# voxelmorph/voxelmorph

Hardware: NVIDIA H100
Metric: vol-pairs/sec (3D 160x192x224 VxmDense int_steps=7 train step, NCC+Grad, Adam) (higher is better)
Workload: dtype bf16 (conv operands) / f32 (accumulate, warp, VecInt, losses)

## Files before the change

include/vxm_b200.h:

```cpp
#ifndef VXM_B200_H
#define VXM_B200_H

#include <stddef.h>
#include <stdint.h>

#ifdef __cplusplus
extern "C" {
#endif

#define VXM_OK 0
#define VXM_ERR_ARG (-1)
#define VXM_ERR_CUDA (-2)
#define VXM_ERR_UNSUPPORTED (-3)

#define VXM_MODE_LINEAR 0
#define VXM_MODE_NEAREST 1
#define VXM_ARITH_TRUE_DIV 0
#define VXM_ARITH_RECIPROCAL 1
#define VXM_ARITH_FAST 2

const char* vxm_last_error(void);
const char* vxm_version(void);
uint64_t vxm_launch_count(void);

int vxm_warp_fwd(const float* src, const float* flow, float* out,
                 int B, int C, int Ds, int Hs, int Ws, int D, int H, int W, int nd,
                 int mode, int arith, void* stream);
int vxm_warp_bwd(const float* grad_out, const float* src, const float* flow,
                 float* grad_src, float* grad_flow,
                 int B, int C, int Ds, int Hs, int Ws, int D, int H, int W, int nd,
                 int mode, int arith, void* stream);

size_t vxm_vecint_workspace_bytes(int B, int D, int H, int W, int nd, int nsteps);
int vxm_vecint_fwd(const float* vel, float* out, float* states, void* work,
                   int B, int D, int H, int W, int nd, int nsteps, int arith, void* stream);
int vxm_vecint_bwd(const float* grad_out, const float* states, float* grad_vel, void* work,
                   int B, int D, int H, int W, int nd, int nsteps, int arith, void* stream);
size_t vxm_vecint_fast_states_bytes(int B, int D, int H, int W, int nsteps);
size_t vxm_vecint_fast_work_bytes(int B, int D, int H, int W, int backward);
int vxm_debug_gridsync(int nsync, int ctas_per_sm, void* stream);

int vxm_resize_fwd(const float* x, float* out, int B, int C, int Di, int Hi, int Wi,
                   int Do, int Ho, int Wo, float pre, float post, void* stream);
int vxm_resize_bwd(const float* grad_out, float* grad_x, int B, int C, int Di, int Hi, int Wi,
                   int Do, int Ho, int Wo, float pre, float post, void* stream);

int vxm_ncc_fwd(const float* I, const float* J, float* loss, float* saved, void* work,
                int B, int D, int H, int W, int wd, int wh, int ww, void* stream);
int vxm_ncc_bwd(const float* I, const float* J, const float* saved, const float* grad_loss,
                float* grad_J, int B, int D, int H, int W, int wd, int wh, int ww, void* stream);
int vxm_ncc_fwd2(const float* I, const float* J, float* loss, float* saved, void* work, int which,
                 int B, int D, int H, int W, int wd, int wh, int ww, void* stream);
int vxm_ncc_bwd2(const float* I, const float* J, const float* saved, const float* grad_loss, float* grad_I,
                 float* grad_J, int which, int B, int D, int H, int W, int wd, int wh, int ww, void* stream);

int vxm_jacdet(const float* disp, float* det, unsigned long long* folds, int B, int D, int H, int W, int nd, void* stream);

size_t vxm_reduce_workspace_bytes(void);
int vxm_gradloss_fwd(const float* y, float* loss, void* work, int B, int C, int D, int H, int W,
                     int nd, int penalty, float mult, void* stream);
int vxm_gradloss_bwd(const float* y, const float* grad_loss, float* grad_y, int B, int C, int D,
                     int H, int W, int nd, int penalty, float mult, void* stream);

int vxm_mse_fwd(const float* y_true, const float* y_pred, float* loss, void* work, size_t n,
                void* stream);
int vxm_mse_bwd(const float* y_true, const float* y_pred, const float* grad_loss,
                float* grad_pred, size_t n, void* stream);
int vxm_mse_scaled_fwd(const float* y_true, const float* y_pred, float* loss, void* work, size_t n, double scale,
                       void* stream);
int vxm_mse_scaled_bwd(const float* y_true, const float* y_pred, const float* grad_loss, float* grad_pred, size_t n,
                       double scale, void* stream);

int vxm_kl_fwd(const float* params, float* loss, void* work, int B, int D, int H, int W, int nd, float prior_lambda,
               void* stream);
int vxm_kl_bwd(const float* params, const float* grad_loss, float* grad_params, int B, int D, int H, int W, int nd,
               float prior_lambda, void* stream);

size_t vxm_dice_workspace_bytes(int BL);
int vxm_dice_fwd(const float* y_true, const float* y_pred, float* loss, float* sums, void* work,
                 int BL, size_t V, void* stream);
int vxm_dice_bwd(const float* y_true, const float* sums, const float* grad_loss, float* grad_pred,
                 int BL, size_t V, void* stream);

int vxm_conv3d_fwd_f32(const float* x, const float* w, const float* bias, float* y,
                       int B, int Cin, int Cout, int D, int H, int W, int kd,
                       float leaky_slope, void* stream);
size_t vxm_conv3d_bwd_workspace_bytes(int B, int Cin, int Cout, int D, int H, int W, int kd);
int vxm_conv3d_bwd_f32(const float* grad_y, const float* y, const float* x, const float* w,
                       float* grad_x, float* grad_w, float* grad_b, void* work,
                       int B, int Cin, int Cout, int D, int H, int W, int kd,
                       float leaky_slope, void* stream);

size_t vxm_conv3d_tc_packed_bytes(int cin_eff, int np, int kd);
int vxm_conv3d_tc_pack(const float* w, void* wpk, int Cout, int Cin, int kd, int np, int transposed,
                       void* stream);
int vxm_conv3d_tc_fwd(const void* xa, const void* xb, const float* const* xf, const long long* xf_bstride,
                      int nplanar, const void* wpk, const float* bias, void* out, const void* mask,
                      int B, int D, int H, int W, int Ca, int Cb, int up, int Cout, int np, int kd,
                      int out_mode, float slope, void* out2, int csplit, void* stream);
size_t vxm_conv3d_tct_packed_bytes(int cin_eff, int coutp, int kd);
int vxm_conv3d_tct_pack(const float* w, void* wpk, int Cout, int Cin, int kd, int coutp, int transposed, void* stream);
int vxm_conv3d_tct_supported(int Ca, int Cb, int Cout);
int vxm_conv3d_tct_fwd(const void* xa, const void* xb, const void* wpk, const float* bias, void* out, const void* mask,
                       int B, int D, int H, int W, int Ca, int Cb, int up, int Cout, int coutp, int kd, int out_mode,
                       float slope, void* out2, int csplit, void* stream);
size_t vxm_conv3d_tcs_packed_bytes(int cin_eff, int coutp, int kd);
int vxm_conv3d_tcs_pack(const float* w, void* wpk, int Cout, int Cin, int kd, int coutp, int transposed, void* stream);
int vxm_conv3d_tcs_supported(int Ca, int Cb, int Cout);
size_t vxm_conv3d_tcs_pack_desc_bytes(void);
int vxm_conv3d_tcs_pack_desc(void* desc_host, const float* w, void* wpk, int Cout, int Cin, int kd, int coutp, int transposed,
                             int begin);
int vxm_conv3d_tcs_pack_desc_blk(void* desc_host, const float* w, void* wpk, int Cout, int Cin, int kd, int coutp, int transposed,
                                 int n0, int nb, int k0, int kb, int begin);
int vxm_conv3d_tcs_pack_desc_fold(void* desc_host, const float* w, void* wpk, int Cout, int Cin, int coutp, int transposed, int begin);
int vxm_conv3d_tcs_pack_multi(const void* descs_dev, int ndesc, int total, void* stream);
int vxm_conv3d_tcs_fwd(const void* xa, const void* xb, const void* wpk, const float* bias, void* out, const void* mask,
                       int B, int D, int H, int W, int Ca, int Cb, int up, int Cout, int coutp, int kd, int out_mode,
                       float slope, void* out2, int csplit, void* stream);
int vxm_conv3d_tcs_fwd_acc(const void* xa, const void* xb, const void* wpk, const float* bias, void* out, void* out_lo,
                           const float* acc_in, int B, int D, int H, int W, int Ca, int Cb, int up, int Cout, int coutp,
                           int kd, int out_mode, float slope, void* stream);
int vxm_conv3d_tcs_fits(int cin, int coutp, int kd);
int vxm_conv3d_tcs_fwd_blk(const void* xa, const void* xb, const void* wpk, const float* bias, void* out, void* out_lo,
                           const void* mask, const float* acc_in, int B, int D, int H, int W, int Ca, int Cb, int up, int Cout,
                           int coutp, int kd, int out_mode, float slope, int opitch, void* stream);
size_t vxm_conv3d_tcs_poly_packed_bytes(int mode, int Cout, int Cin, int Ca);
int vxm_conv3d_tcs_pack_desc_poly(void* desc_host, const float* w, void* wpk, int Cout, int Cin, int Ca, int mode, int begin);
int vxm_conv3d_tcs_poly(const void* xa, const void* xb, const void* wpk, const float* bias, void* out, const void* mask, int B, int D,
                        int H, int W, int Ca, int Cb, int Cout, int mode, float slope, void* stream);
size_t vxm_conv3d_tc_wgrad_workspace_bytes(int kd);
int vxm_conv3d_tc_wgrad(const void* xa, const void* xb, const float* const* xf, const long long* xf_bstride,
                        int nplanar_x, const void* gz, const float* const* gf, const long long* gf_bstride,
                        int nplanar_g, float* grad_w, float* grad_b, void* work, int B, int D, int H, int W,
                        int Ca, int Cb, int up, int Cin_real, int Cg, int Cout_real, int kd, int accumulate, void* stream);
size_t vxm_conv3d_tc_wgrad2_desc_bytes(void);
int vxm_conv3d_tc_wgrad2_max_pending(void);
size_t vxm_conv3d_tc_wgrad2_partial_bytes(int kd);
int vxm_conv3d_tc_wgrad2_partial(const void* xa, const void* xb, const void* gz, float* grad_w, float* grad_b, void* work,
                                 size_t work_bytes, size_t* work_used, void* descs_host, int* ndesc, int B, int D, int H, int W,
                                 int Ca, int Cb, int up, int Cin_real, int Cg, int Cout_real, int kd, int accumulate, void* stream);
int vxm_conv3d_tc_wgrad2_flush(const void* descs_host, int ndesc, void* stream);
int vxm_conv3d_tc_wgrad2_partial_khm(const void* x, const void* gz, float* grad_w, float* grad_b, void* work, size_t work_bytes,
                                     size_t* work_used, void* descs_host, int* ndesc, int B, int D, int H, int W, int Cx,
                                     int Cin_real, int Cg, int Cout_real, int accumulate, void* stream);
int vxm_pool2_ndhwc_bf16(const void* x_fine, void* y_coarse, int B, int Dc, int Hc, int Wc, int C, int nd, void* stream);
int vxm_sumpool_mask_ndhwc_bf16(const void* g_fine, const void* act_coarse, void* out_coarse, int B, int Dc, int Hc,
                                int Wc, int C, int nd, float slope, void* stream);
int vxm_unpool_combine_ndhwc_bf16(const void* e_fine, const void* g_skip_fine, const void* g_pool_coarse, void* out_fine,
                                  int B, int Dc, int Hc, int Wc, int C, int nd, float slope, void* stream);
int vxm_planar_to_ndhwc8_bf16(const float* const* planes, const long long* bstrides, int nplanes, void* out, int B,
                              size_t V, void* stream);
int vxm_planar_fold_kd_bf16(const float* const* planes, const long long* bstrides, int nplanes, void* out, int B, int D,
                            size_t HW, int cout, void* stream);
int vxm_planar_to_ndhwc8_split_bf16(const float* const* planes, const long long* bstrides, int nplanes, void* out_hi,
                                    void* out_lo, int B, size_t V, void* stream);
int vxm_pool2_split_ndhwc_bf16(const void* x_hi, const void* x_lo, void* y_hi, void* y_lo, int B, int Dc, int Hc, int Wc,
                               int C, int nd, void* stream);
int vxm_unpool_combine_split_ndhwc_bf16(const void* e_hi, const void* e_lo, const void* g_skip_fine, const void* g_pool_coarse,
                                        void* out_fine, int B, int Dc, int Hc, int Wc, int C, int nd, float slope, void* stream);

int vxm_maxpool2_fwd(const float* x, float* y, uint8_t* idx, int B, int C, int D, int H, int W,
                     int nd, void* stream);
int vxm_maxpool2_bwd(const float* grad_y, const uint8_t* idx, float* grad_x, int B, int C, int D,
                     int H, int W, int nd, void* stream);
int vxm_upcat_fwd(const float* a, const float* skip, float* out, int B, int Ca, int Cb, int D,
                  int H, int W, int nd, void* stream);
int vxm_upcat_bwd(const float* grad_out, float* grad_a, float* grad_skip, int B, int Ca, int Cb,
                  int D, int H, int W, int nd, void* stream);

int vxm_adam_step(float* p, const float* g, float* m, float* v, size_t n, int step, float lr,
                  float beta1, float beta2, float eps, float weight_decay, float grad_scale,
                  void* stream);

int vxm_adam_step_dev(float* p, const float* g, float* m, float* v, size_t n, int* step_counter, float lr,
                      float beta1, float beta2, float eps, float weight_decay, float grad_scale, void* stream);

int vxm_mean_stream_fwd(const float* x, float* mean, float* count, float* out, float* saved, void* work, int B, size_t n,
                        float cap, int commit, void* stream);
int vxm_mean_stream_bwd(const float* grad_out, const float* saved, float* grad_x, int B, size_t n, size_t gout_bstride,
                        void* stream);

int vxm_sample_normal_logvar_fwd(const float* params, float* z, long long* state, long long* ticket, void* work, int B,
                                 int nd, size_t V, void* stream);
int vxm_sample_normal_logvar_bwd(const float* grad_z, const float* params, const long long* state, const long long* ticket,
                                 float* grad_params, int B, int nd, size_t V, void* stream);

size_t vxm_pheno_decoder_workspace_bytes(int F);
int vxm_pheno_decoder_fwd(const float* pheno, const float* W, const float* bias, const float* like_w, const float* like_b,
                          float* out, int B, int P, int F, size_t V, void* stream);
int vxm_pheno_decoder_bwd(const float* grad_out, const float* pheno, const float* W, const float* bias, const float* like_w,
                          float* grad_W, float* grad_bias, float* grad_like_w, float* grad_like_b, void* work, int B, int P,
                          int F, size_t V, int accumulate, void* stream);

size_t vxm_hyper_workspace_bytes(int U, size_t N);
int vxm_hyper_mlp_fwd(const float* hyp, const float* const* weights, const float* const* biases, float* pre, float* h,
                      int P, int U, int nb_layers, void* stream);
int vxm_hyper_mlp_bwd(const float* grad_h, const float* hyp, const float* const* weights, const float* pre,
                      float* const* grad_weights, float* const* grad_biases, int P, int U, int nb_layers, int accumulate,
                      void* stream);
int vxm_hyper_weights_fwd(const float* h, const float* A, const float* a, float* W, int U, size_t N, void* stream);
int vxm_hyper_weights_bwd(const float* h, const float* A, const float* grad_W, float* grad_A, float* grad_a,
                          float* grad_h, void* work, int U, size_t N, int accumulate, void* stream);

size_t vxm_mi_workspace_bytes(int N, size_t V, int nbins);
int vxm_mi_fwd(const float* y_true, const float* y_pred, const float* centers, float* loss, void* work, void* reduce_work,
               int N, size_t V, int nbins, float alpha, float min_clip, float max_clip, void* stream);
int vxm_mi_bwd(const float* y_true, const float* y_pred, const float* centers, const float* grad_loss, float* grad_true,
               float* grad_pred, void* work, int N, size_t V, int nbins, float alpha, float min_clip, float max_clip,
               void* stream);

size_t vxm_point_warp_workspace_bytes(int B, int N, int D, int H, int W, int nd);
int vxm_point_warp_fwd(const float* points, const float* flow, float* out, int B, int N, int D, int H, int W, int nd,
                       float r, void* stream);
int vxm_point_warp_bwd(const float* points, const float* grad_out, float* grad_flow, void* work, size_t work_bytes,
                       int B, int N, int D, int H, int W, int nd, float r, void* stream);
int vxm_value_at_fwd(const float* sdt, const float* points, float* out, int B, int N, int L, int D, int H, int W,
                     int nd, void* stream);
int vxm_value_at_bwd(const float* sdt, const float* points, const float* grad_out, float* grad_points, int B, int N,
                     int L, int D, int H, int W, int nd, void* stream);

#ifdef __cplusplus
}
#endif
#endif
```

voxelmorph_b200/_lib.py:

```python
import ctypes
import os
import threading

import torch

_HERE = os.path.dirname(os.path.abspath(__file__))
LIB_PATH = os.path.join(_HERE, "libvxm_b200.so")

c_f = ctypes.c_void_p
c_i = ctypes.c_int
c_sz = ctypes.c_size_t
c_fl = ctypes.c_float
c_d = ctypes.c_double

SIGNATURES = {
    "vxm_last_error": (ctypes.c_char_p, []),
    "vxm_version": (ctypes.c_char_p, []),
    "vxm_launch_count": (ctypes.c_uint64, []),
    "vxm_warp_fwd": (c_i, [c_f, c_f, c_f] + [c_i] * 9 + [c_i, c_i, c_f]),
    "vxm_warp_bwd": (c_i, [c_f, c_f, c_f, c_f, c_f] + [c_i] * 9 + [c_i, c_i, c_f]),
    "vxm_vecint_workspace_bytes": (c_sz, [c_i] * 6),
    "vxm_vecint_fwd": (c_i, [c_f, c_f, c_f, c_f] + [c_i] * 7 + [c_f]),
    "vxm_vecint_bwd": (c_i, [c_f, c_f, c_f, c_f] + [c_i] * 7 + [c_f]),
    "vxm_vecint_fast_states_bytes": (c_sz, [c_i] * 5),
    "vxm_vecint_fast_work_bytes": (c_sz, [c_i] * 5),
    "vxm_debug_gridsync": (c_i, [c_i, c_i, c_f]),
    "vxm_resize_fwd": (c_i, [c_f, c_f] + [c_i] * 8 + [c_fl, c_fl, c_f]),
    "vxm_resize_bwd": (c_i, [c_f, c_f] + [c_i] * 8 + [c_fl, c_fl, c_f]),
    "vxm_ncc_fwd": (c_i, [c_f, c_f, c_f, c_f, c_f] + [c_i] * 7 + [c_f]),
    "vxm_ncc_bwd": (c_i, [c_f, c_f, c_f, c_f, c_f] + [c_i] * 7 + [c_f]),
    "vxm_ncc_fwd2": (c_i, [c_f, c_f, c_f, c_f, c_f] + [c_i] * 8 + [c_f]),
    "vxm_ncc_bwd2": (c_i, [c_f, c_f, c_f, c_f, c_f, c_f] + [c_i] * 8 + [c_f]),
    "vxm_jacdet": (c_i, [c_f, c_f, c_f] + [c_i] * 5 + [c_f]),
    "vxm_reduce_workspace_bytes": (c_sz, []),
    "vxm_gradloss_fwd": (c_i, [c_f, c_f, c_f] + [c_i] * 7 + [c_fl, c_f]),
    "vxm_gradloss_bwd": (c_i, [c_f, c_f, c_f] + [c_i] * 7 + [c_fl, c_f]),
    "vxm_mse_fwd": (c_i, [c_f, c_f, c_f, c_f, c_sz, c_f]),
    "vxm_mse_bwd": (c_i, [c_f, c_f, c_f, c_f, c_sz, c_f]),
    "vxm_mse_scaled_fwd": (c_i, [c_f, c_f, c_f, c_f, c_sz, c_d, c_f]),
    "vxm_mse_scaled_bwd": (c_i, [c_f, c_f, c_f, c_f, c_sz, c_d, c_f]),
    "vxm_kl_fwd": (c_i, [c_f, c_f, c_f] + [c_i] * 5 + [c_fl, c_f]),
    "vxm_kl_bwd": (c_i, [c_f, c_f, c_f] + [c_i] * 5 + [c_fl, c_f]),
    "vxm_dice_workspace_bytes": (c_sz, [c_i]),
    "vxm_dice_fwd": (c_i, [c_f, c_f, c_f, c_f, c_f, c_i, c_sz, c_f]),
    "vxm_dice_bwd": (c_i, [c_f, c_f, c_f, c_f, c_i, c_sz, c_f]),
    "vxm_conv3d_fwd_f32": (c_i, [c_f, c_f, c_f, c_f] + [c_i] * 7 + [c_fl, c_f]),
    "vxm_conv3d_bwd_workspace_bytes": (c_sz, [c_i] * 7),
    "vxm_conv3d_bwd_f32": (c_i, [c_f] * 8 + [c_i] * 7 + [c_fl, c_f]),
    "vxm_conv3d_tc_packed_bytes": (c_sz, [c_i] * 3),
    "vxm_conv3d_tc_pack": (c_i, [c_f, c_f] + [c_i] * 5 + [c_f]),
    "vxm_conv3d_tc_fwd": (c_i, [c_f, c_f, c_f, c_f, c_i, c_f, c_f, c_f, c_f] + [c_i] * 11 + [c_fl, c_f, c_i, c_f]),
    "vxm_conv3d_tct_packed_bytes": (c_sz, [c_i] * 3),
    "vxm_conv3d_tct_pack": (c_i, [c_f, c_f] + [c_i] * 5 + [c_f]),
    "vxm_conv3d_tct_supported": (c_i, [c_i] * 3),
    "vxm_conv3d_tct_fwd": (c_i, [c_f, c_f, c_f, c_f, c_f, c_f] + [c_i] * 11 + [c_fl, c_f, c_i, c_f]),
    "vxm_conv3d_tcs_packed_bytes": (c_sz, [c_i] * 3),
    "vxm_conv3d_tcs_pack": (c_i, [c_f, c_f] + [c_i] * 5 + [c_f]),
    "vxm_conv3d_tcs_supported": (c_i, [c_i] * 3),
    "vxm_conv3d_tcs_pack_desc_bytes": (c_sz, []),
    "vxm_conv3d_tcs_pack_desc": (c_i, [c_f, c_f, c_f] + [c_i] * 6),
    "vxm_conv3d_tcs_pack_desc_blk": (c_i, [c_f, c_f, c_f] + [c_i] * 10),
    "vxm_conv3d_tcs_pack_desc_fold": (c_i, [c_f, c_f, c_f] + [c_i] * 5),
    "vxm_conv3d_tcs_pack_multi": (c_i, [c_f, c_i, c_i, c_f]),
    "vxm_conv3d_tcs_fwd": (c_i, [c_f, c_f, c_f, c_f, c_f, c_f] + [c_i] * 11 + [c_fl, c_f, c_i, c_f]),
    "vxm_conv3d_tcs_fwd_acc": (c_i, [c_f, c_f, c_f, c_f, c_f, c_f, c_f] + [c_i] * 11 + [c_fl, c_f]),
    "vxm_conv3d_tcs_fits": (c_i, [c_i] * 3),
    "vxm_conv3d_tcs_fwd_blk": (c_i, [c_f] * 8 + [c_i] * 11 + [c_fl, c_i, c_f]),
    "vxm_conv3d_tcs_poly_packed_bytes": (c_sz, [c_i] * 4),
    "vxm_conv3d_tcs_pack_desc_poly": (c_i, [c_f, c_f, c_f] + [c_i] * 5),
    "vxm_conv3d_tcs_poly": (c_i, [c_f] * 6 + [c_i] * 8 + [c_fl, c_f]),
    "vxm_conv3d_tc_wgrad_workspace_bytes": (c_sz, [c_i]),
    "vxm_conv3d_tc_wgrad": (c_i, [c_f, c_f, c_f, c_f, c_i, c_f, c_f, c_f, c_i, c_f, c_f, c_f] + [c_i] * 12 + [c_f]),
    "vxm_conv3d_tc_wgrad2_desc_bytes": (c_sz, []),
    "vxm_conv3d_tc_wgrad2_max_pending": (c_i, []),
    "vxm_conv3d_tc_wgrad2_partial_bytes": (c_sz, [c_i]),
    "vxm_conv3d_tc_wgrad2_partial": (c_i, [c_f, c_f, c_f, c_f, c_f, c_f, c_sz, c_f, c_f, c_f] + [c_i] * 12 + [c_f]),
    "vxm_conv3d_tc_wgrad2_flush": (c_i, [c_f, c_i, c_f]),
    "vxm_conv3d_tc_wgrad2_partial_khm": (c_i, [c_f, c_f, c_f, c_f, c_f, c_sz, c_f, c_f, c_f] + [c_i] * 9 + [c_f]),
    "vxm_pool2_ndhwc_bf16": (c_i, [c_f, c_f] + [c_i] * 6 + [c_f]),
    "vxm_sumpool_mask_ndhwc_bf16": (c_i, [c_f, c_f, c_f] + [c_i] * 6 + [c_fl, c_f]),
    "vxm_unpool_combine_ndhwc_bf16": (c_i, [c_f, c_f, c_f, c_f] + [c_i] * 6 + [c_fl, c_f]),
    "vxm_planar_to_ndhwc8_bf16": (c_i, [c_f, c_f, c_i, c_f, c_i, c_sz, c_f]),
    "vxm_planar_to_ndhwc8_split_bf16": (c_i, [c_f, c_f, c_i, c_f, c_f, c_i, c_sz, c_f]),
    "vxm_planar_fold_kd_bf16": (c_i, [c_f, c_f, c_i, c_f, c_i, c_i, c_sz, c_i, c_f]),
    "vxm_pool2_split_ndhwc_bf16": (c_i, [c_f, c_f, c_f, c_f] + [c_i] * 6 + [c_f]),
    "vxm_unpool_combine_split_ndhwc_bf16": (c_i, [c_f, c_f, c_f, c_f, c_f] + [c_i] * 6 + [c_fl, c_f]),
    "vxm_maxpool2_fwd": (c_i, [c_f, c_f, c_f] + [c_i] * 6 + [c_f]),
    "vxm_maxpool2_bwd": (c_i, [c_f, c_f, c_f] + [c_i] * 6 + [c_f]),
    "vxm_upcat_fwd": (c_i, [c_f, c_f, c_f] + [c_i] * 7 + [c_f]),
    "vxm_upcat_bwd": (c_i, [c_f, c_f, c_f] + [c_i] * 7 + [c_f]),
    "vxm_adam_step": (c_i, [c_f, c_f, c_f, c_f, c_sz, c_i] + [c_fl] * 6 + [c_f]),
    "vxm_adam_step_dev": (c_i, [c_f, c_f, c_f, c_f, c_sz, c_f] + [c_fl] * 6 + [c_f]),
    "vxm_mean_stream_fwd": (c_i, [c_f] * 6 + [c_i, c_sz, c_fl, c_i, c_f]),
    "vxm_mean_stream_bwd": (c_i, [c_f, c_f, c_f, c_i, c_sz, c_sz, c_f]),
    "vxm_sample_normal_logvar_fwd": (c_i, [c_f] * 5 + [c_i, c_i, c_sz, c_f]),
    "vxm_sample_normal_logvar_bwd": (c_i, [c_f] * 5 + [c_i, c_i, c_sz, c_f]),
    "vxm_pheno_decoder_workspace_bytes": (c_sz, [c_i]),
    "vxm_pheno_decoder_fwd": (c_i, [c_f] * 6 + [c_i, c_i, c_i, c_sz, c_f]),
    "vxm_pheno_decoder_bwd": (c_i, [c_f] * 10 + [c_i, c_i, c_i, c_sz, c_i, c_f]),
    "vxm_hyper_workspace_bytes": (c_sz, [c_i, c_sz]),
    "vxm_hyper_mlp_fwd": (c_i, [c_f] * 5 + [c_i, c_i, c_i, c_f]),
    "vxm_hyper_mlp_bwd": (c_i, [c_f] * 6 + [c_i, c_i, c_i, c_i, c_f]),
    "vxm_hyper_weights_fwd": (c_i, [c_f] * 4 + [c_i, c_sz, c_f]),
    "vxm_hyper_weights_bwd": (c_i, [c_f] * 7 + [c_i, c_sz, c_i, c_f]),
    "vxm_mi_workspace_bytes": (c_sz, [c_i, c_sz, c_i]),
    "vxm_mi_fwd": (c_i, [c_f] * 6 + [c_i, c_sz, c_i, c_fl, c_fl, c_fl, c_f]),
    "vxm_mi_bwd": (c_i, [c_f] * 7 + [c_i, c_sz, c_i, c_fl, c_fl, c_fl, c_f]),
    "vxm_point_warp_workspace_bytes": (c_sz, [c_i] * 6),
    "vxm_point_warp_fwd": (c_i, [c_f] * 3 + [c_i] * 6 + [c_fl, c_f]),
    "vxm_point_warp_bwd": (c_i, [c_f] * 4 + [c_sz] + [c_i] * 6 + [c_fl, c_f]),
    "vxm_value_at_fwd": (c_i, [c_f] * 3 + [c_i] * 7 + [c_f]),
    "vxm_value_at_bwd": (c_i, [c_f] * 4 + [c_i] * 7 + [c_f]),
}

_lib = None
_lock = threading.Lock()


class VxmError(RuntimeError):
    pass


def load():
    global _lib
    if _lib is not None:
        return _lib
    with _lock:
        if _lib is not None:
            return _lib
        if not os.path.isfile(LIB_PATH):
            raise VxmError(
                "voxelmorph_b200: %s not found — build it with `python -c 'import __graft_entry__ as g; g.build()'` "
                "(or `make -C voxelmorph_b200/csrc`).  There is no CPU / torch fallback." % LIB_PATH)
        lib = ctypes.CDLL(LIB_PATH)
        for name, (res, args) in SIGNATURES.items():
            fn = getattr(lib, name)
            fn.restype = res
            fn.argtypes = args
        _lib = lib
    return _lib


def last_error():
    return load().vxm_last_error().decode("utf-8", "replace")


def check(rc, what):
    if rc != 0:
        raise VxmError("%s failed (%d): %s" % (what, rc, last_error()))


def launch_count():
    return int(load().vxm_launch_count())


def ptr(t):
    if t is None:
        return None
    return ctypes.c_void_p(t.data_ptr())


def stream_ptr():
    return ctypes.c_void_p(torch.cuda.current_stream().cuda_stream)


def require_cuda(*tensors, what="voxelmorph_b200"):
    for t in tensors:
        if t is None:
            continue
        if not t.is_cuda:
            raise VxmError("%s: CUDA tensors are required (the GPU path has no CPU fallback); got a %s tensor"
                           % (what, t.device))
        if t.dtype != torch.float32:
            raise VxmError("%s: float32 tensors are required at the module boundary; got %s" % (what, t.dtype))


def contig(t):
    return t if t.is_contiguous() else t.contiguous()


_reduce_ws = {}


def reduce_workspace(device):
    key = (device.index, torch.cuda.current_stream(device).cuda_stream)
    ws = _reduce_ws.get(key)
    if ws is None:
        lib = load()
        with _lock:
            ws = _reduce_ws.get(key)
            if ws is None:
                nbytes = int(lib.vxm_reduce_workspace_bytes())
                ws = torch.zeros(nbytes, dtype=torch.uint8, device=device)
                _reduce_ws[key] = ws
    return ws
```

voxelmorph_b200/csrc/conv3d_tc_s.cu:

```cuda
#include <stdlib.h>
#include <string.h>

#include "tc_common.cuh"

namespace vxm {
namespace tcs {

using namespace vxm::tc;

constexpr int WT = 32, WUSE = 30;
constexpr int MAXSLOT = 16;
constexpr int NLOADER = 128, NTHREADS = 384, NGRP = 2;

struct ConvSArgs {
  const __nv_bfloat16* xa; const __nv_bfloat16* xb;
  const __nv_bfloat16* wpk; const float* bias;
  void* out; const __nv_bfloat16* mask;
  void* out2; int csplit;
  int B, D, H, W, Ca, Cb, up, upd, Cout, out_mode;
  float slope;
  int tiles_h, tiles_w, dchunk, nchunks, nitems, nslot;
  uint32_t wbytes;
  const float* acc_in; void* out_lo;
  int tma_mask, tc0[2];
  int opitch;
  alignas(64) CUtensorMap tm[2];
};

__host__ __device__ inline uint32_t swz(uint32_t off, uint32_t width) {
  return off ^ (((off >> 7) & (width / 16 - 1)) << 4);
}
__device__ __forceinline__ uint64_t make_desc_kmajor_swz(uint32_t saddr, uint32_t width) {
  uint64_t d = 0;
  d |= (uint64_t)((saddr >> 4) & 0x3FFF);
  d |= (uint64_t)1 << 16;
  d |= (uint64_t)(((8u * width) >> 4) & 0x3FFF) << 32;
  return d | desc_swizzle(width);
}

__device__ __forceinline__ void named_bar_arrive(int id, int nthreads) {
  asm volatile("bar.arrive %0, %1;" ::"r"(id), "r"(nthreads) : "memory");
}

template <int KD, int G0, int G1, int COUT, int HT, bool ACC, int EPI, bool OP = false, int PD = 0>
__global__ void __launch_bounds__(NTHREADS, 1) conv_tcs_kernel(const __grid_constant__ ConvSArgs a) {
  static_assert(PD == 0 || (KD == 3 && EPI != 0 && !ACC && !OP), "polyphase forms: 3-D, specialised epilogue");
  static_assert(PD != 1 || G1 > 0, "the polyphase forward merges channel group 0 and keeps group 1");
  static_assert(PD != 2 || (G1 == 0 && COUT == 32 && HT == 8 && EPI == 2), "the coarse dgrad: 32 -> 32 channels, 8-row tiles");
  static_assert(EPI != 4 || (PD == 0 && !ACC && !OP && COUT <= 32), "the fp32 planar epilogue drains in the fragment layout");
  static_assert(KD == 3 || EPI == 0 || (EPI != 3 && COUT <= 32), "KD = 1: fragment-layout epilogues 1, 2, 4 only");
  constexpr int SROWS = (HT + 2) * WT;
  constexpr int NH = PD == 2 ? 1 : HT / 4;
  constexpr int NEVEN = (HT + 3) / 2;
  constexpr int W0 = G0 * 2, W1 = G1 * 2;
  constexpr int NC8 = (G0 + G1) / 8;
  constexpr uint32_t SLAB0 = SROWS * W0, SLAB1 = SROWS * W1;
  constexpr int NN = 3 * COUT;
  extern __shared__ __align__(1024) uint8_t smem[];
  const bool halfk = (a.Ca + a.Cb == 8);
  constexpr uint32_t slab_bytes = SLAB0 + SLAB1;
  const int NSLOT = a.nslot;
  uint8_t* s_w = smem;
  uint8_t* s_slab = smem + ((a.wbytes + 1023u) & ~1023u);
  float* s_stage = reinterpret_cast<float*>(s_slab + NSLOT * slab_bytes);
  uint64_t* bars = reinterpret_cast<uint64_t*>(s_stage + NGRP * ACC_STAGE_FLOATS);
  uint64_t* full = bars;
  uint64_t* empty = bars + MAXSLOT;
  uint64_t* wbar = empty + MAXSLOT;

  const int warp = threadIdx.x >> 5, lane = threadIdx.x & 31;

  const bool tma0 = a.tma_mask & 1, tma1 = (a.tma_mask & 2) != 0;
  const bool all_tma = tma0 && (G1 == 0 || tma1);
  if (threadIdx.x == 0) {
    for (int i = 0; i < NSLOT; ++i) { mbar_init(&full[i], all_tma ? 1 : NLOADER); mbar_init(&empty[i], 4 * NGRP); }
    mbar_init(wbar, 1);
    fence_barrier_init();
  }
  __syncthreads();

  if (threadIdx.x == 0) {
    mbar_expect_tx(wbar, a.wbytes);
    for (uint32_t off = 0; off < a.wbytes; off += 16384u) {
      uint32_t n = a.wbytes - off < 16384u ? a.wbytes - off : 16384u;
      bulk_g2s(s_w + off, reinterpret_cast<const uint8_t*>(a.wpk) + off, n, wbar);
    }
  }
  const int HW_tiles = a.tiles_h * a.tiles_w;
  const int Dout = PD == 2 ? a.D >> 1 : a.D;

  if (warp >= 8) {
    const int lt = threadIdx.x - 8 * 32;
    uint32_t slot = 0, lphase = 1;
    const int Da = a.upd ? a.D >> 1 : a.D, Ha = a.up ? a.H >> 1 : a.H, Wa = a.up ? a.W >> 1 : a.W;
    const int nca8 = a.Ca >> 3;
    constexpr int nchunk = NC8 * SROWS;
    constexpr int KMAX = (nchunk + NLOADER - 1) / NLOADER;
    if (lt == 0) {
      if (tma0) tma_prefetch_desc(&a.tm[0]);
      if (tma1) tma_prefetch_desc(&a.tm[1]);
    }
    const uint32_t tma_bytes = (tma0 ? SLAB0 : 0u) + (tma1 ? SLAB1 : 0u);
    for (int item = blockIdx.x; item < a.nitems && !(all_tma && lt != 0); item += gridDim.x) {
      const int wt = item % a.tiles_w, ht = (item / a.tiles_w) % a.tiles_h;
      const int ch = (item / HW_tiles) % a.nchunks, b = item / (HW_tiles * a.nchunks);
      const int h0 = ht * HT, w0 = wt * WUSE, d0 = ch * a.dchunk, d1 = min(d0 + a.dchunk, Dout);
      const int s_begin = PD == 2 ? 2 * d0 - 1 : (KD == 3 ? d0 - 1 : d0), s_end = PD == 2 ? 2 * d1 + 1 : (KD == 3 ? d1 + 1 : d1);
      int soff[KMAX];
      uint32_t doff[KMAX];
#pragma unroll
      for (int k = 0; k < KMAX; ++k) {
        const int id = lt + k * NLOADER;
        soff[k] = -1;
        doff[k] = 0;
        if (id < nchunk) {
          const int c8 = id % NC8, row = id / NC8;
          const int r = row >> 5, c = row & 31;
          const int h = h0 - 1 + r, w = w0 - 1 + c;
          const int srow = PD == 2 ? ((r & 1) ? NEVEN + (r >> 1) : (r >> 1)) * WT + c : row;
          doff[k] = c8 < G0 / 8 ? swz((uint32_t)srow * W0 + (uint32_t)c8 * 16u, W0)
                                : SLAB0 + swz((uint32_t)row * W1 + (uint32_t)(c8 - G0 / 8) * 16u, W1 ? W1 : 32);
          if (c8 < G0 / 8 ? tma0 : tma1) soff[k] = -2;
          else if (h >= 0 && h < a.H && w >= 0 && w < a.W && !(halfk && c8 > 0)) {
            if (c8 < nca8) soff[k] = (((a.up ? h >> 1 : h) * Wa + (a.up ? w >> 1 : w)) * a.Ca + c8 * 8) << 1;
            else soff[k] = (((h * a.W + w) * a.Cb + (c8 - nca8) * 8) << 1) | 1;
          }
        }
      }
      for (int ds = s_begin; ds < s_end; ++ds) {
        mbar_wait(&empty[slot], lphase);
        uint8_t* slab = s_slab + (size_t)slot * slab_bytes;
        const bool dok = ds >= 0 && ds < a.D;
        const __nv_bfloat16* baseA = a.xa ? a.xa + (((size_t)b * Da + (dok ? (a.upd ? ds >> 1 : ds) : 0)) * Ha * Wa) * a.Ca : nullptr;
        const __nv_bfloat16* baseB = a.xb ? a.xb + (((size_t)b * a.D + (dok ? ds : 0)) * a.H * a.W) * a.Cb : nullptr;
        const __nv_bfloat16* dummy = a.xa ? a.xa : a.xb;
        if (lt == 0 && tma_bytes) {
          if (all_tma) mbar_expect_tx(&full[slot], tma_bytes);
          else mbar_expect_tx_noarrive(&full[slot], tma_bytes);
          if (tma0) tma_load_5d(slab, &a.tm[0], a.tc0[0], w0 - 1, h0 - 1, ds, b, &full[slot]);
          if (tma1) tma_load_5d(slab + SLAB0, &a.tm[1], a.tc0[1], w0 - 1, h0 - 1, ds, b, &full[slot]);
        }
        if (!all_tma) {
#pragma unroll
          for (int k = 0; k < KMAX; ++k) {
            if (lt + k * NLOADER < nchunk && soff[k] != -2) {
              const bool ok = dok && soff[k] >= 0;
              const __nv_bfloat16* src = ok ? ((soff[k] & 1) ? baseB : baseA) + (soff[k] >> 1) : dummy;
              cp_async16(slab + doff[k], src, ok ? 16u : 0u);
            }
          }
          cp_async_arrive_noinc(&full[slot]);
        }
        if (++slot == (uint32_t)NSLOT) { slot = 0; lphase ^= 1; }
      }
    }
  } else {
    const int grp = warp >> 2;
    const int wq = warp & 3;
    float* stage = s_stage + grp * ACC_STAGE_FLOATS;
    const int nbar = 1 + grp;
    constexpr int NSUB = NN > 96 ? 2 : 1;
    constexpr int NF = 2 / NSUB;
    constexpr int NCH = NSUB == 1 ? COUT / 16 : (COUT + 31) / 32;
    const int trow0 = NSUB == 1 ? wq : (wq & 1);
    auto chan = [&](int i) { return NSUB == 1 ? 16 * i : 32 * i + 16 * (wq >> 1); };
    const uint32_t slab_u32 = smem_u32(s_slab), w_u32 = smem_u32(s_w);
    constexpr uint32_t WSTEP = (uint32_t)NN * (W0 + W1);
    mbar_wait(wbar, 0);
    const uint64_t bdesc0 = make_desc_kmajor_swz(w_u32, W0);
    const uint64_t bdesc1 = make_desc_kmajor_swz(w_u32 + NN * W0, W1 ? W1 : 32);
    uint32_t cnt_base = 0, ecnt = 0, wcur = 0;
    auto observe = [&](uint32_t upto) {
      for (; wcur <= upto; ++wcur) mbar_wait(&full[wcur % NSLOT], (wcur / NSLOT) & 1);
    };
    constexpr int NKD = PD == 2 ? 4 : KD;
    auto mma = [&](uint32_t hslot, int hb, int sub, float (&acc)[NF][NN / 2], int par) {
      uint64_t adesc0_kd[NKD], adesc1_kd[NKD];
      uint32_t sl = hslot;
#pragma unroll
      for (int kd = 0; kd < NKD; ++kd) {
        adesc0_kd[kd] = make_desc_kmajor_swz(slab_u32 + sl * slab_bytes, W0);
        adesc1_kd[kd] = make_desc_kmajor_swz(slab_u32 + sl * slab_bytes + SLAB0, W1 ? W1 : 32);
        if (++sl == (uint32_t)NSLOT) sl = 0;
      }
      wg_fence();
#pragma unroll
      for (int kd = 0; kd < NKD; ++kd) {
#pragma unroll
        for (int kh = 0; kh < (PD == 2 ? 4 : 3); ++kh) {
          const int st = kd * (PD == 2 ? 4 : 3) + kh;
#pragma unroll
          for (int k = 0; k < (G0 + G1) / 16; ++k) {
            const bool g0 = k < G0 / 16;
            if (PD == 1 && g0 && kd == 2) continue;
            const int kk = g0 ? k : k - G0 / 16;
            const uint32_t wr = g0 ? W0 : W1;
            uint64_t abase = g0 ? adesc0_kd[kd] : adesc1_kd[kd];
            uint32_t wst = st * WSTEP;
            if (PD == 1 && g0 && par) {
              abase = adesc0_kd[kd + 1 < NKD ? kd + 1 : kd];
              wst = kd == 0 ? 9 * WSTEP + kh * NN * W0 : (6 + kh) * WSTEP;
            }
            const int r0 = PD == 2 ? ((kh & 1) ? NEVEN : 0) + (kh >> 1) : hb * 4 + kh;
            const uint64_t adesc = abase + (uint64_t)((r0 * WT * wr + kk * 32) >> 4);
            const uint64_t bdesc = (g0 ? bdesc0 : bdesc1) + (uint64_t)((wst + kk * 32) >> 4);
#pragma unroll
            for (int f = 0; f < NF; ++f)
              Wgmma<NN, 0, 0>::mma(acc[f], adesc + (uint64_t)(((sub + f) * 2 * WT * wr) >> 4), bdesc, (st | k) ? 1u : 0u);
          }
        }
      }
      wg_commit();
    };
    auto readout = [&](float (&acc)[NF][NN / 2], int c, uint32_t (&r)[16]) {
      if constexpr (NSUB == 1) acc_row16(acc[0], acc[NF - 1], c, stage, nbar, r);
      else acc_half_row16(acc[0], c, COUT - (c % COUT) < 32 ? 16 : 32, stage, nbar, r);
    };
    auto combine = [&](float (&acc)[NF][NN / 2], int i, float (&v)[16]) {
      const int cb = NSUB == 1 ? 16 * i : 32 * i;
      uint32_t r[16];
      readout(acc, cb, r);
#pragma unroll
      for (int c = 0; c < 16; ++c) v[c] = __shfl_up_sync(0xffffffffu, __uint_as_float(r[c]), 1);
      readout(acc, COUT + cb, r);
#pragma unroll
      for (int c = 0; c < 16; ++c) v[c] += __uint_as_float(r[c]);
      readout(acc, 2 * COUT + cb, r);
#pragma unroll
      for (int c = 0; c < 16; ++c) v[c] += __shfl_down_sync(0xffffffffu, __uint_as_float(r[c]), 1);
    };
    auto release = [&](int nd) {
      if (KD == 3) {
        const uint32_t last = PD == 2 ? 2u * nd : (uint32_t)nd;
        observe(cnt_base + last + 1u);
        if (lane == 0) {
          mbar_arrive(&empty[(cnt_base + last) % NSLOT]);
          mbar_arrive(&empty[(cnt_base + last + 1) % NSLOT]);
        }
        cnt_base += last + 2;
      } else {
        cnt_base += nd;
      }
    };
    if constexpr (EPI != 0) {
      const float slope = a.slope;
      const int c1 = (EPI == 3 && a.out2) ? a.csplit : COUT;
      const int Ho = PD == 2 ? a.H >> 1 : a.H, Wo = PD == 2 ? a.W >> 1 : a.W;
      const size_t HWp = (size_t)Ho * Wo;
      const int q = lane >> 2, p = lane & 3, half = wq & 1, pair = wq >> 1;
      const int xbar = 3 + 2 * grp + pair;
      constexpr bool ROWS = NSUB > 1 || PD == 2;
      constexpr int XPAIR = NF * 2 * COUT;
      static_assert(2 * 2 * XPAIR <= ACC_STAGE_FLOATS, "seam exchange fits the stage buffer");
      uint32_t xpar = 0;
      constexpr bool ORD = !ROWS;
      [[maybe_unused]] uint32_t nev = 0;
      if constexpr (ORD) {
        for (int item = blockIdx.x; item < a.nitems; item += gridDim.x) {
          const int d0 = ((item / HW_tiles) % a.nchunks) * a.dchunk;
          nev += (uint32_t)(min(d0 + a.dchunk, Dout) - d0) * NH;
        }
        if (grp == 1) named_bar_arrive(7, 256);
      }
      for (int item = blockIdx.x; item < a.nitems; item += gridDim.x) {
        const int wt = item % a.tiles_w, ht = (item / a.tiles_w) % a.tiles_h;
        const int ch = (item / HW_tiles) % a.nchunks, b = item / (HW_tiles * a.nchunks);
        const int d0 = ch * a.dchunk, d1 = min(d0 + a.dchunk, Dout);
        const int nd = d1 - d0;
        const int wp = 16 * half + q, w = wt * WUSE - 1 + wp;
        const int hbase = ht * HT + pair;
        uint32_t okm = 0;
#pragma unroll
        for (int hb = 0; hb < NH; ++hb)
#pragma unroll
          for (int blk = 0; blk < 2; ++blk)
#pragma unroll
            for (int i = 0; i < 2; ++i)
              if (wp + 8 * i >= 1 && wp + 8 * i <= WUSE && w + 8 * i < a.W && hbase + 4 * hb + 2 * blk < Ho)
                okm |= 1u << (4 * hb + 2 * blk + i);
        size_t vbase = (((size_t)b * Dout + d0) * Ho + hbase) * Wo + (size_t)(long long)w;
        [[maybe_unused]] const size_t DHWp = (size_t)Dout * HWp, pbase = (size_t)b * (a.Cout - 1) * DHWp;
        for (int j = 0; j < nd; ++j) {
          const uint32_t js = PD == 2 ? 2u * j : (uint32_t)j;
          observe(cnt_base + js + (PD == 2 ? 3u : (KD == 3 ? 2u : 0u)));
          const uint32_t hslot = (cnt_base + js) % NSLOT;
#pragma unroll
          for (int hb = 0; hb < NH; ++hb) {
            if ((int)(ecnt++ % NGRP) != grp) continue;
            auto vox_of = [&](int blk, int i) { return vbase + (size_t)((4 * hb + 2 * blk) * Wo + 8 * i); };
#pragma unroll
            for (int sub = 0; sub < NSUB; ++sub) {
              [[maybe_unused]] uint32_t mreg[EPI == 2 && !ROWS ? NF : 1][2][COUT / 8];
              auto load_mask = [&](int f) {
                if constexpr (EPI == 2 && !ROWS) {
#pragma unroll
                  for (int i = 0; i < 2; ++i)
                    if (okm >> (4 * hb + 2 * f + i) & 1u) {
                      const uint32_t* mp = reinterpret_cast<const uint32_t*>(a.mask + vox_of(f, i) * (OP ? a.opitch : COUT) + 2 * p);
#pragma unroll
                      for (int jj = 0; jj < COUT / 8; ++jj) mreg[f][i][jj] = __ldg(mp + 4 * jj);
                    }
                }
              };
              if constexpr (COUT == 16) {
#pragma unroll
                for (int f = 0; f < NF; ++f) load_mask(f);
              }
              const int rh = PD == 2 ? ht * (HT / 2) + trow0 : ht * HT + hb * 4 + trow0 + 2 * sub, rw = wt * WUSE - 1 + lane;
              const bool rvalid = lane >= 1 && lane <= WUSE && rw < a.W && rh < Ho && (PD != 2 || (lane & 1));
              const size_t rvox = (((size_t)b * Dout + d0 + j) * Ho + rh) * Wo + (PD == 2 ? rw >> 1 : rw);
              [[maybe_unused]] uint32_t mrow[PD == 2 ? NCH : 1][8];
              if constexpr (PD == 2) {
#pragma unroll
                for (int i = 0; i < NCH; ++i)
                  if (rvalid) ld_global_nc_v8(a.mask + rvox * COUT + chan(i), mrow[i]);
              }
              float acc[NF][NN / 2];
              [[maybe_unused]] const uint32_t e = ecnt - 1;
              if constexpr (ORD) named_bar(7 + grp, 256);
              mma(hslot, hb, sub, acc, (d0 + j) & 1);
              if (ORD && e + 1 < nev) named_bar_arrive(8 - grp, 256);
              wg_wait<0>();
              if constexpr (ROWS) {
                const bool valid = rvalid;
                const size_t vox = rvox;
#pragma unroll
                for (int i = 0; i < NCH; ++i) {
                  const int c0 = chan(i);
                  float v[16];
                  combine(acc, i, v);
                  if (c0 >= COUT) continue;
                  if constexpr (PD == 2) {
#pragma unroll
                    for (int c = 0; c < 16; ++c) v[c] += __shfl_down_sync(0xffffffffu, v[c], 1);
                  }
                  if constexpr (EPI == 1) {
#pragma unroll
                    for (int c = 0; c < 16; ++c) {
                      const float x = v[c] + (a.bias ? __ldg(a.bias + c0 + c) : 0.f);
                      v[c] = fmaxf(x, x * slope);
                    }
                  } else if constexpr (EPI == 2) {
                    uint32_t mreg[8];
                    if constexpr (PD == 2) {
#pragma unroll
                      for (int e = 0; e < 8; ++e) mreg[e] = mrow[i][e];
                    } else if (valid) {
                      ld_global_nc_v8(a.mask + vox * (OP ? a.opitch : COUT) + c0, mreg);
                    }
#pragma unroll
                    for (int e = 0; e < 8; ++e) {
                      if (mreg[e] & 0x8000u) v[2 * e] *= slope;
                      if (mreg[e] & 0x80000000u) v[2 * e + 1] *= slope;
                    }
                  }
                  if (valid) {
                    __nv_bfloat16* dst = (EPI == 3 && c0 >= c1) ? reinterpret_cast<__nv_bfloat16*>(a.out2) + vox * (COUT - c1) + (c0 - c1)
                                                                : reinterpret_cast<__nv_bfloat16*>(a.out) + vox * (OP ? a.opitch : c1) + c0;
                    st_global_v8(dst, pack_bf16x2(v[0], v[1]), pack_bf16x2(v[2], v[3]), pack_bf16x2(v[4], v[5]), pack_bf16x2(v[6], v[7]),
                                 pack_bf16x2(v[8], v[9]), pack_bf16x2(v[10], v[11]), pack_bf16x2(v[12], v[13]), pack_bf16x2(v[14], v[15]));
                  }
                }
                continue;
              }
              float* xb = stage + xpar * (2 * XPAIR) + pair * XPAIR;
              xpar ^= 1u;
              if (half == 0 ? q == 7 : q == 0) {
#pragma unroll
                for (int f = 0; f < NF; ++f)
#pragma unroll
                  for (int jj = 0; jj < COUT / 8; ++jj) {
                    float2* xs = reinterpret_cast<float2*>(xb + f * 2 * COUT + 8 * jj + 2 * p);
                    const int k0 = 4 * jj + 2, k2 = 4 * (COUT / 4 + jj);
                    if (half == 0) xs[0] = make_float2(acc[f][k0], acc[f][k0 + 1]);
                    else xs[COUT / 2] = make_float2(acc[f][k2], acc[f][k2 + 1]);
                  }
              }
              named_bar(xbar, 64);
#pragma unroll
              for (int f = 0; f < NF; ++f) {
                const int blk = sub + f;
                if constexpr (COUT != 16) load_mask(f);
#pragma unroll
                for (int jj = 0; jj < COUT / 8; ++jj) {
                  if (EPI == 4 && 8 * jj >= a.Cout) break;
                  const int c0 = 8 * jj + 2 * p;
                  float v[2][2];
#pragma unroll
                  for (int e = 0; e < 2; ++e) {
                    const float* xs = xb + f * 2 * COUT + c0 + e;
                    const int k0 = 4 * jj + e, k1 = 4 * (COUT / 8 + jj) + e, k2 = 4 * (COUT / 4 + jj) + e;
                    const float a1 = __shfl_sync(0xffffffffu, q == 7 ? acc[f][k0] : acc[f][k0 + 2], (lane + 28) & 31);
                    const float a0 = __shfl_sync(0xffffffffu, acc[f][k0], (lane + 28) & 31);
                    const float b0 = __shfl_sync(0xffffffffu, q == 0 ? acc[f][k2 + 2] : acc[f][k2], (lane + 4) & 31);
                    const float b1 = __shfl_sync(0xffffffffu, acc[f][k2 + 2], (lane + 4) & 31);
                    float x0 = q == 0 ? xs[0] : a0;
                    x0 += acc[f][k1];
                    x0 += b0;
                    float x1 = a1;
                    x1 += acc[f][k1 + 2];
                    x1 += q == 7 ? xs[COUT] : b1;
                    v[0][e] = x0;
                    v[1][e] = x1;
                  }
#pragma unroll
                  for (int i = 0; i < 2; ++i) {
                    if constexpr (EPI == 1) {
#pragma unroll
                      for (int e = 0; e < 2; ++e) {
                        const float x = v[i][e] + (a.bias ? __ldg(a.bias + c0 + e) : 0.f);
                        v[i][e] = fmaxf(x, x * slope);
                      }
                    } else if constexpr (EPI == 2 && KD == 3) {
                      const uint32_t mw = mreg[f][i][jj];
                      if (mw & 0x8000u) v[i][0] *= slope;
                      if (mw & 0x80000000u) v[i][1] *= slope;
                    } else if constexpr (EPI == 2) {
                      const uint32_t mw = mreg[f][i][jj];
                      v[i][0] += 0.f;
                      v[i][1] += 0.f;
                      if (__uint_as_float(mw << 16) < 0.f) v[i][0] *= slope;
                      if (__uint_as_float(mw & 0xffff0000u) < 0.f) v[i][1] *= slope;
                    } else if constexpr (EPI == 4) {
#pragma unroll
                      for (int e = 0; e < 2; ++e) {
                        float x = v[i][e] + (a.bias && c0 + e < a.Cout ? __ldg(a.bias + c0 + e) : 0.f);
                        if (slope >= 0.f) x = x >= 0.f ? x : x * slope;
                        v[i][e] = x;
                      }
                    }
                    if constexpr (EPI == 4) {
                      if (okm >> (4 * hb + 2 * blk + i) & 1u) {
                        float* o = reinterpret_cast<float*>(a.out) + vox_of(blk, i) + pbase + (size_t)c0 * DHWp;
                        if (c0 < a.Cout) o[0] = v[i][0];
                        if (c0 + 1 < a.Cout) o[DHWp] = v[i][1];
                      }
                    } else if (okm >> (4 * hb + 2 * blk + i) & 1u) {
                      const size_t vox = vox_of(blk, i);
                      __nv_bfloat16* dst = (EPI == 3 && c0 >= c1) ? reinterpret_cast<__nv_bfloat16*>(a.out2) + vox * (COUT - c1) + (c0 - c1)
                                                                  : reinterpret_cast<__nv_bfloat16*>(a.out) + vox * (OP ? a.opitch : c1) + c0;
                      *reinterpret_cast<uint32_t*>(dst) = pack_bf16x2(v[i][0], v[i][1]);
                    }
                  }
                }
              }
            }
          }
          vbase += HWp;
          if (lane == 0) {
            mbar_arrive(&empty[hslot]);
            if (PD == 2) mbar_arrive(&empty[(hslot + 1) % NSLOT]);
          }
        }
        release(nd);
      }
    } else {
    const size_t HWp = (size_t)a.H * a.W;
    auto bias_at = [&](int c) -> float { return a.bias ? __ldg(a.bias + c) : 0.f; };
    for (int item = blockIdx.x; item < a.nitems; item += gridDim.x) {
      const int wt = item % a.tiles_w, ht = (item / a.tiles_w) % a.tiles_h;
      const int ch = (item / HW_tiles) % a.nchunks, b = item / (HW_tiles * a.nchunks);
      const int w = wt * WUSE - 1 + lane, d0 = ch * a.dchunk, d1 = min(d0 + a.dchunk, a.D);
      const int nd = d1 - d0;
      for (int j = 0; j < nd; ++j) {
        const int d = d0 + j;
        observe(cnt_base + (uint32_t)j + (KD == 3 ? 2u : 0u));
        const uint32_t hslot = (cnt_base + j) % NSLOT;
#pragma unroll
        for (int hb = 0; hb < NH; ++hb) {
        if ((int)(ecnt++ % NGRP) != grp) continue;
#pragma unroll
        for (int sub = 0; sub < NSUB; ++sub) {
        const int h = ht * HT + hb * 4 + trow0 + 2 * sub;
        const bool valid = lane >= 1 && lane <= WUSE && h < a.H && w < a.W;
        const size_t vox = (((size_t)b * a.D + d) * a.H + h) * a.W + w;
        constexpr bool PREF = NSUB == 1;
        [[maybe_unused]] uint4 mreg[PREF ? NCH : 1][2];
        if (PREF && a.mask && valid) {
#pragma unroll
          for (int i = 0; i < NCH; ++i)
#pragma unroll
            for (int q = 0; q < 2; ++q)
              if (chan(i) + 8 * q < a.Cout)
                mreg[i][q] = __ldg(reinterpret_cast<const uint4*>(a.mask + vox * (OP ? a.opitch : a.Cout) + chan(i)) + q);
        }
        const int c1 = a.out2 ? a.csplit : a.Cout;
        float acc[NF][NN / 2];
        mma(hslot, hb, sub, acc, 0);
        wg_wait<0>();
#pragma unroll
        for (int i = 0; i < NCH; ++i) {
          const int c0 = chan(i);
          [[maybe_unused]] float4 ain[ACC ? 4 : 1];
          if constexpr (ACC && !OP && PREF) {
            if (a.acc_in && valid && c0 < COUT) {
              const float4* ap = reinterpret_cast<const float4*>(a.acc_in + vox * COUT + c0);
#pragma unroll
              for (int q = 0; q < 4; ++q) ain[q] = __ldg(ap + q);
            }
          }
          float v[16];
          combine(acc, i, v);
          if (NSUB > 1 && c0 >= COUT) continue;
          bool handled = false;
          if constexpr (ACC) {
            if (a.acc_in && valid) {
              if constexpr (OP || !PREF) {
                const float4* ap = reinterpret_cast<const float4*>(a.acc_in + vox * COUT + c0);
#pragma unroll
                for (int q = 0; q < 4; ++q) ain[q] = __ldg(ap + q);
              }
#pragma unroll
              for (int q = 0; q < 4; ++q) { v[4 * q] += ain[q].x; v[4 * q + 1] += ain[q].y; v[4 * q + 2] += ain[q].z; v[4 * q + 3] += ain[q].w; }
            }
            if (a.out_mode == 2) {
              handled = true;
              if (valid) {
                float4* op = reinterpret_cast<float4*>(reinterpret_cast<float*>(a.out) + vox * COUT + c0);
#pragma unroll
                for (int q = 0; q < 4; ++q) op[q] = make_float4(v[4 * q], v[4 * q + 1], v[4 * q + 2], v[4 * q + 3]);
              }
            } else if (a.out_mode == 3) {
              handled = true;
              if (valid && c0 < a.Cout) {
#pragma unroll
                for (int q = 0; q < 16; q += 8) {
                  if (c0 + q < a.Cout) {
                    uint32_t hi[4], lo[4];
#pragma unroll
                    for (int e = 0; e < 8; e += 2) {
                      float x0 = v[q + e] + bias_at(c0 + q + e), x1 = v[q + e + 1] + bias_at(c0 + q + e + 1);
                      if (a.slope >= 0.f) { x0 = x0 >= 0.f ? x0 : x0 * a.slope; x1 = x1 >= 0.f ? x1 : x1 * a.slope; }
                      const __nv_bfloat16 h0 = __float2bfloat16_rn(x0), h1 = __float2bfloat16_rn(x1);
                      hi[e >> 1] = (uint32_t)__bfloat16_as_ushort(h0) | ((uint32_t)__bfloat16_as_ushort(h1) << 16);
                      lo[e >> 1] = pack_bf16x2(x0 - __bfloat162float(h0), x1 - __bfloat162float(h1));
                    }
                    const size_t o = vox * (OP ? a.opitch : a.Cout) + c0 + q;
                    *reinterpret_cast<uint4*>(reinterpret_cast<__nv_bfloat16*>(a.out) + o) = make_uint4(hi[0], hi[1], hi[2], hi[3]);
                    *reinterpret_cast<uint4*>(reinterpret_cast<__nv_bfloat16*>(a.out_lo) + o) = make_uint4(lo[0], lo[1], lo[2], lo[3]);
                  }
                }
              }
            }
          }
          if (!handled && valid && c0 < a.Cout) {
            if (a.out_mode == 0) {
#pragma unroll
              for (int q = 0; q < 16; q += 8) {
                if (c0 + q < a.Cout) {
                  float x[8];
#pragma unroll
                  for (int e = 0; e < 8; ++e) x[e] = v[q + e] + bias_at(c0 + q + e);
                  if (a.mask) {
                    uint4 m4;
                    if constexpr (PREF) m4 = mreg[i][q / 8];
                    else m4 = __ldg(reinterpret_cast<const uint4*>(a.mask + vox * (OP ? a.opitch : a.Cout) + c0) + q / 8);
                    const __nv_bfloat16* mb = reinterpret_cast<const __nv_bfloat16*>(&m4);
#pragma unroll
                    for (int e = 0; e < 8; ++e) if (__bfloat162float(mb[e]) < 0.f) x[e] *= a.slope;
                  } else if (a.slope >= 0.f) {
#pragma unroll
                    for (int e = 0; e < 8; ++e) x[e] = x[e] >= 0.f ? x[e] : x[e] * a.slope;
                  }
                  const int cg = c0 + q;
                  __nv_bfloat16* oo = cg < c1 ? reinterpret_cast<__nv_bfloat16*>(a.out) + vox * (OP ? a.opitch : c1) + cg
                                              : reinterpret_cast<__nv_bfloat16*>(a.out2) + vox * (a.Cout - c1) + (cg - c1);
                  *reinterpret_cast<uint4*>(oo) = make_uint4(pack_bf16x2(x[0], x[1]), pack_bf16x2(x[2], x[3]), pack_bf16x2(x[4], x[5]), pack_bf16x2(x[6], x[7]));
                }
              }
            } else {
              float* o = reinterpret_cast<float*>(a.out);
#pragma unroll
              for (int c = 0; c < 16; ++c) {
                if (c0 + c < a.Cout) {
                  float x = v[c] + bias_at(c0 + c);
                  if (a.slope >= 0.f) x = x >= 0.f ? x : x * a.slope;
                  o[(((size_t)b * a.Cout + c0 + c) * a.D + d) * HWp + (size_t)h * a.W + w] = x;
                }
              }
            }
          }
        }
        }
        }
        if (lane == 0) mbar_arrive(&empty[hslot]);
      }
      release(nd);
    }
    }
  }
}

__global__ void pack_weights_s_kernel(const float* __restrict__ w, __nv_bfloat16* __restrict__ out, int Cout, int Cin, int KD, int COUT,
                                      int NN, int G0, int G1, int transposed) {
  const int T = KD * 9;
  const int CG = G0 + G1;
  const int total = KD * 3 * NN * CG;
  for (int i = blockIdx.x * blockDim.x + threadIdx.x; i < total; i += gridDim.x * blockDim.x) {
    const int ci = i % CG, n = (i / CG) % NN, st = i / (CG * NN);
    const int kd = st / 3, kh = st % 3, g = n / COUT, co = n % COUT;
    const int tap = (kd * 3 + kh) * 3 + g;
    float v = 0.f;
    if (!transposed) {
      if (co < Cout && ci < Cin) v = w[((size_t)co * Cin + ci) * T + tap];
    } else {
      if (co < Cin && ci < Cout) v = w[((size_t)ci * Cin + co) * T + (T - 1 - tap)];
    }
    const uint32_t W0 = G0 * 2, W1 = G1 * 2;
    uint32_t off;
    if (ci < G0) off = swz((uint32_t)n * W0 + (uint32_t)ci * 2u, W0);
    else off = (uint32_t)NN * W0 + swz((uint32_t)n * W1 + (uint32_t)(ci - G0) * 2u, W1);
    out[((size_t)st * NN * (W0 + W1) + off) / 2] = __float2bfloat16_rn(v);
  }
}

struct PackDesc {
  const float* w;
  __nv_bfloat16* out;
  int Cout, Cin, KD, COUT, NN, G0, G1, transposed;
  int begin, count;
  int fold;
  int n0, nb, k0, kb;
  int poly;
};
__global__ void pack_weights_multi_kernel(const PackDesc* __restrict__ descs, int ndesc, int total) {
  for (int gi = blockIdx.x * blockDim.x + threadIdx.x; gi < total; gi += gridDim.x * blockDim.x) {
    int lo = 0, hi = ndesc - 1;
    while (lo < hi) {
      const int mid = (lo + hi + 1) >> 1;
      if (descs[mid].begin <= gi) lo = mid; else hi = mid - 1;
    }
    const PackDesc d = descs[lo];
    const int i = gi - d.begin;
    const int T = d.KD * 9, CG = d.G0 + d.G1;
    const int base = d.KD * 3 * d.NN * CG;
    const bool extra = d.poly == 1 && i >= base;
    const int ie = i - base;
    const int ci = extra ? ie % d.G0 : i % CG, n = extra ? (ie / d.G0) % d.NN : (i / CG) % d.NN;
    const int st = extra ? ie / (d.G0 * d.NN) : i / (CG * d.NN);
    const int kd = extra ? 0 : (d.poly == 2 ? st >> 2 : st / 3), kh = extra ? st : (d.poly == 2 ? st & 3 : st % 3);
    const int g = n / d.COUT, co = n % d.COUT;
    const int tap = (kd * 3 + kh) * 3 + g;
    float v = 0.f;
    if (d.poly) {
      if (co < d.nb && ci < d.kb) {
        int t0 = kd, t1 = kd, u0 = kh, u1 = kh;
        if (d.poly == 1 && ci < d.G0) t1 = extra ? 1 : (kd == 1 ? 2 : kd);
        if (d.poly == 2) {
          t0 = kd > 0 ? kd - 1 : 0; t1 = kd < 2 ? kd : 2;
          u0 = kh > 0 ? kh - 1 : 0; u1 = kh < 2 ? kh : 2;
        }
        for (int t = t0; t <= t1; ++t)
          for (int u = u0; u <= u1; ++u) {
            const int tp = (t * 3 + u) * 3 + g;
            v += !d.transposed ? d.w[((size_t)(d.n0 + co) * d.Cin + d.k0 + ci) * 27 + tp]
                               : d.w[((size_t)(d.k0 + ci) * d.Cin + d.n0 + co) * 27 + (26 - tp)];
          }
      }
    } else if (d.fold) {
      const int fk = ci / d.fold, c = ci % d.fold;
      const int tap3 = (fk * 3 + kh) * 3 + g;
      if (fk < 3) {
        if (!d.transposed) { if (co < d.Cout) v = d.w[((size_t)co * d.Cin + c) * 27 + tap3]; }
        else if (co < d.Cin) v = d.w[((size_t)c * d.Cin + co) * 27 + (26 - tap3)];
      }
    } else if (co < d.nb && ci < d.kb) {
      if (!d.transposed) v = d.w[((size_t)(d.n0 + co) * d.Cin + d.k0 + ci) * T + tap];
      else v = d.w[((size_t)(d.k0 + ci) * d.Cin + d.n0 + co) * T + (T - 1 - tap)];
    }
    const uint32_t W0 = d.G0 * 2, W1 = d.G1 * 2;
    uint32_t off;
    if (extra) off = (uint32_t)base * 2u + (uint32_t)(st * d.NN) * W0 + swz((uint32_t)n * W0 + (uint32_t)ci * 2u, W0);
    else if (ci < d.G0) off = (uint32_t)(st * d.NN) * (W0 + W1) + swz((uint32_t)n * W0 + (uint32_t)ci * 2u, W0);
    else off = (uint32_t)(st * d.NN) * (W0 + W1) + (uint32_t)d.NN * W0 + swz((uint32_t)n * W1 + (uint32_t)(ci - d.G0) * 2u, W1);
    d.out[off / 2] = __float2bfloat16_rn(v);
  }
}

static void groups_of(int cin, int* g0, int* g1) {
  if (cin == 8 || cin == 16) { *g0 = 16; *g1 = 0; }
  else if (cin == 32) { *g0 = 32; *g1 = 0; }
  else if (cin == 48) { *g0 = 32; *g1 = 16; }
  else { *g0 = 64; *g1 = 0; }
}

static int plan_tma(ConvSArgs& a, int g0, int g1, int HTv) {
  a.tma_mask = 0;
  a.tc0[0] = a.tc0[1] = 0;
  const char* e = getenv("VXM_B200_TMA");
  if (e && e[0] == '0') return 0;
  const int lo[2] = {0, g0}, hi[2] = {g0, g0 + g1};
  for (int g = 0; g < 2; ++g) {
    if (hi[g] == lo[g]) continue;
    const void* base = nullptr;
    int C = 0, c0 = 0;
    if (a.xa && hi[g] <= a.Ca && !a.up) { base = a.xa; C = a.Ca; c0 = lo[g]; }
    else if (a.xb && lo[g] >= a.Ca && hi[g] <= a.Ca + a.Cb) { base = a.xb; C = a.Cb; c0 = lo[g] - a.Ca; }
    if (!base) continue;
    if (tc::make_act_tmap(&a.tm[g], base, a.B, a.D, a.H, a.W, C, hi[g] - lo[g], WT, HTv + 2) != 0) return -1;
    a.tma_mask |= 1 << g;
    a.tc0[g] = c0;
  }
  return 0;
}

}
}

using namespace vxm;
using namespace vxm::tcs;

extern "C" size_t vxm_conv3d_tcs_packed_bytes(int cin_eff, int coutp, int kd) {
  int g0, g1;
  groups_of(cin_eff <= 8 ? 8 : (cin_eff <= 16 ? 16 : (cin_eff <= 32 ? 32 : (cin_eff <= 48 ? 48 : 64))), &g0, &g1);
  return (size_t)kd * 3 * (3 * coutp) * (g0 + g1) * sizeof(__nv_bfloat16);
}

extern "C" int vxm_conv3d_tcs_pack(const float* w, void* wpk, int Cout, int Cin, int kd, int coutp, int transposed, void* stream) {
  VXM_REQUIRE(w && wpk && Cout > 0 && Cin > 0 && (kd == 1 || kd == 3) && (coutp == 16 || coutp == 32 || coutp == 48 || coutp == 64), "conv3d_tcs_pack: bad argument");
  int cin_eff = transposed ? Cout : Cin, nout = transposed ? Cin : Cout;
  VXM_REQUIRE(nout <= coutp, "conv3d_tcs_pack: %d output channels do not fit %d", nout, coutp);
  VXM_REQUIRE(cin_eff <= 64, "conv3d_tcs_pack: at most 64 input channels");
  int g0, g1;
  groups_of(cin_eff <= 8 ? 8 : (cin_eff <= 16 ? 16 : (cin_eff <= 32 ? 32 : (cin_eff <= 48 ? 48 : 64))), &g0, &g1);
  int NN = 3 * coutp;
  int total = kd * 3 * NN * (g0 + g1);
  pack_weights_s_kernel<<<(total + 255) / 256, 256, 0, as_stream(stream)>>>(w, (__nv_bfloat16*)wpk, Cout, Cin, kd, coutp, NN, g0, g1, transposed);
  return check_launch("conv3d_tcs_pack");
}

extern "C" size_t vxm_conv3d_tcs_pack_desc_bytes(void) { return sizeof(PackDesc); }

extern "C" int vxm_conv3d_tcs_pack_desc_blk(void* desc_host, const float* w, void* wpk, int Cout, int Cin, int kd, int coutp, int transposed,
                                            int n0, int nb, int k0, int kb, int begin) {
  VXM_REQUIRE(desc_host && w && wpk && Cout > 0 && Cin > 0 && (kd == 1 || kd == 3) && (coutp == 16 || coutp == 32 || coutp == 48 || coutp == 64),
              "conv3d_tcs_pack_desc: bad argument");
  const int cin_eff = transposed ? Cout : Cin, nout = transposed ? Cin : Cout;
  VXM_REQUIRE(n0 >= 0 && nb > 0 && n0 + nb <= nout && k0 >= 0 && kb > 0 && k0 + kb <= cin_eff, "conv3d_tcs_pack_desc: block out of range");
  VXM_REQUIRE(nb <= coutp && kb <= 64, "conv3d_tcs_pack_desc: channel counts do not fit");
  int g0, g1;
  groups_of(kb <= 8 ? 8 : (kb <= 16 ? 16 : (kb <= 32 ? 32 : (kb <= 48 ? 48 : 64))), &g0, &g1);
  PackDesc d;
  d.w = w; d.out = (__nv_bfloat16*)wpk; d.Cout = Cout; d.Cin = Cin; d.KD = kd; d.COUT = coutp; d.NN = 3 * coutp; d.G0 = g0; d.G1 = g1;
  d.transposed = transposed; d.begin = begin; d.count = kd * 3 * d.NN * (g0 + g1); d.fold = 0;
  d.n0 = n0; d.nb = nb; d.k0 = k0; d.kb = kb; d.poly = 0;
  memcpy(desc_host, &d, sizeof(d));
  return d.count;
}

extern "C" int vxm_conv3d_tcs_pack_desc(void* desc_host, const float* w, void* wpk, int Cout, int Cin, int kd, int coutp, int transposed,
                                        int begin) {
  VXM_REQUIRE(Cout > 0 && Cin > 0, "conv3d_tcs_pack_desc: bad argument");
  return vxm_conv3d_tcs_pack_desc_blk(desc_host, w, wpk, Cout, Cin, kd, coutp, transposed, 0, transposed ? Cin : Cout, 0,
                                      transposed ? Cout : Cin, begin);
}

extern "C" int vxm_conv3d_tcs_pack_desc_fold(void* desc_host, const float* w, void* wpk, int Cout, int Cin, int coutp, int transposed, int begin) {
  VXM_REQUIRE(desc_host && w && wpk && Cout > 0 && Cin > 0 && (coutp == 16 || coutp == 32), "conv3d_tcs_pack_desc_fold: bad argument");
  const int real_in = transposed ? Cout : Cin, nout = transposed ? Cin : Cout;
  VXM_REQUIRE(3 * real_in <= 16 && nout <= coutp, "conv3d_tcs_pack_desc_fold: %d x 3 input channels / %d outputs do not fit", real_in, nout);
  int g0, g1;
  groups_of(3 * real_in <= 8 ? 8 : 16, &g0, &g1);
  PackDesc d;
  d.w = w; d.out = (__nv_bfloat16*)wpk; d.Cout = Cout; d.Cin = Cin; d.KD = 1; d.COUT = coutp; d.NN = 3 * coutp; d.G0 = g0; d.G1 = g1;
  d.transposed = transposed; d.begin = begin; d.count = 3 * d.NN * (g0 + g1); d.fold = real_in;
  d.n0 = d.nb = d.k0 = d.kb = 0; d.poly = 0;
  memcpy(desc_host, &d, sizeof(d));
  return d.count;
}

static int poly_geometry(int mode, int Cout, int Cin, int Ca, int* g0, int* g1, int* kd, int* coutp) {
  if (mode == 1 && Ca == 32 && Cin == 48 && Cout == 32) { *g0 = 32; *g1 = 16; *kd = 3; *coutp = 32; return 1; }
  if (mode == 2 && Ca == 32 && Cin > Ca && Cout == 32) { *g0 = 32; *g1 = 0; *kd = 4; *coutp = 32; return 1; }
  return 0;
}

static size_t poly_bytes(int mode) {
  const size_t NN = 3 * 32;
  return (mode == 1 ? 9 * NN * (32 + 16) + 3 * NN * 32 : 16 * NN * 32) * sizeof(__nv_bfloat16);
}

extern "C" size_t vxm_conv3d_tcs_poly_packed_bytes(int mode, int Cout, int Cin, int Ca) {
  int g0, g1, kd, coutp;
  return poly_geometry(mode, Cout, Cin, Ca, &g0, &g1, &kd, &coutp) ? poly_bytes(mode) : 0;
}

extern "C" int vxm_conv3d_tcs_pack_desc_poly(void* desc_host, const float* w, void* wpk, int Cout, int Cin, int Ca, int mode, int begin) {
  int g0, g1, kd, coutp;
  VXM_REQUIRE(desc_host && w && wpk && poly_geometry(mode, Cout, Cin, Ca, &g0, &g1, &kd, &coutp),
              "conv3d_tcs_pack_desc_poly: no polyphase operand for mode %d, (%d of %d) -> %d", mode, Ca, Cin, Cout);
  PackDesc d;
  d.w = w; d.out = (__nv_bfloat16*)wpk; d.Cout = Cout; d.Cin = Cin; d.KD = kd; d.COUT = coutp; d.NN = 3 * coutp; d.G0 = g0; d.G1 = g1;
  d.transposed = mode == 2; d.begin = begin; d.fold = 0; d.poly = mode;
  d.n0 = 0; d.nb = mode == 1 ? Cout : Ca; d.k0 = 0; d.kb = mode == 1 ? Cin : Cout;
  d.count = (int)(vxm_conv3d_tcs_poly_packed_bytes(mode, Cout, Cin, Ca) / sizeof(__nv_bfloat16));
  memcpy(desc_host, &d, sizeof(d));
  return d.count;
}

extern "C" int vxm_conv3d_tcs_pack_multi(const void* descs_dev, int ndesc, int total, void* stream) {
  VXM_REQUIRE(descs_dev && ndesc > 0 && total > 0, "conv3d_tcs_pack_multi: bad argument");
  const int blocks = (total + 255) / 256, cap = sm_count() * 8;
  pack_weights_multi_kernel<<<blocks < cap ? blocks : cap, 256, 0, as_stream(stream)>>>((const PackDesc*)descs_dev, ndesc, total);
  return check_launch("conv3d_tcs_pack_multi");
}

extern "C" int vxm_conv3d_tcs_supported(int Ca, int Cb, int Cout) {
  int cin = Ca + Cb;
  bool split_ok = cin != 48 || (Ca == 32 && Cb == 16) || Cb == 0 || Ca == 0;
  return (Cout <= 64) && (cin == 8 || cin == 16 || cin == 32 || cin == 48 || cin == 64) && Ca % 8 == 0 && Cb % 8 == 0 && split_ok;
}

static int conv_tcs_launch(const void* xa, const void* xb, const void* wpk, const float* bias, void* out, const void* mask,
                           int B, int D, int H, int W, int Ca, int Cb, int up, int Cout, int coutp, int kd, int out_mode,
                           float slope, void* out2, int csplit, const float* acc_in, void* out_lo, int opitch, int poly,
                           void* stream);

extern "C" int vxm_conv3d_tcs_poly(const void* xa, const void* xb, const void* wpk, const float* bias, void* out, const void* mask, int B,
                                   int D, int H, int W, int Ca, int Cb, int Cout, int mode, float slope, void* stream) {
  VXM_REQUIRE(mode == 1 || mode == 2, "conv3d_tcs_poly: mode must be 1 (forward) or 2 (coarse dgrad)");
  return conv_tcs_launch(xa, xb, wpk, bias, out, mask, B, D, H, W, Ca, Cb, mode == 1 ? 1 : 0, Cout, 32, 3, 0, slope, nullptr, 0,
                         nullptr, nullptr, 0, mode, stream);
}

static size_t fixed_smem(uint32_t wbytes) { return ((wbytes + 1023u) & ~1023u) + NGRP * ACC_STAGE_FLOATS * sizeof(float) + 1024 + 512; }

extern "C" int vxm_conv3d_tcs_fits(int cin, int coutp, int kd) {
  int g0, g1;
  groups_of(cin <= 8 ? 8 : (cin <= 16 ? 16 : (cin <= 32 ? 32 : (cin <= 48 ? 48 : 64))), &g0, &g1);
  const size_t slab4 = (size_t)6 * WT * (g0 + g1) * 2;
  return fixed_smem((uint32_t)vxm_conv3d_tcs_packed_bytes(cin, coutp, kd)) + 4 * slab4 <= 227 * 1024;
}

extern "C" int vxm_conv3d_tcs_fwd(const void* xa, const void* xb, const void* wpk, const float* bias, void* out, const void* mask,
                                  int B, int D, int H, int W, int Ca, int Cb, int up, int Cout, int coutp, int kd, int out_mode,
                                  float slope, void* out2, int csplit, void* stream) {
  VXM_REQUIRE(out_mode == 0 || out_mode == 1, "conv3d_tcs_fwd: out_mode must be 0 (bf16 channels-last) or 1 (fp32 planar)");
  return conv_tcs_launch(xa, xb, wpk, bias, out, mask, B, D, H, W, Ca, Cb, up, Cout, coutp, kd, out_mode, slope, out2, csplit,
                         nullptr, nullptr, 0, 0, stream);
}

extern "C" int vxm_conv3d_tcs_fwd_blk(const void* xa, const void* xb, const void* wpk, const float* bias, void* out, void* out_lo,
                                      const void* mask, const float* acc_in, int B, int D, int H, int W, int Ca, int Cb, int up, int Cout,
                                      int coutp, int kd, int out_mode, float slope, int opitch, void* stream) {
  VXM_REQUIRE(out_mode == 0 || out_mode == 2 || out_mode == 3, "conv3d_tcs_fwd_blk: out_mode must be 0 (bf16), 2 (fp32 partial sums) or 3 (bf16 hi/lo pair)");
  VXM_REQUIRE(out_mode != 3 || out_lo, "conv3d_tcs_fwd_blk: out_mode 3 needs out_lo");
  VXM_REQUIRE(opitch == 0 || (opitch >= Cout && opitch % 8 == 0 && out_mode != 2), "conv3d_tcs_fwd_blk: bad output pitch %d", opitch);
  return conv_tcs_launch(xa, xb, wpk, bias, out, mask, B, D, H, W, Ca, Cb, up, Cout, coutp, kd, out_mode, slope, nullptr, 0,
                         acc_in, out_lo, opitch == Cout ? 0 : opitch, 0, stream);
}

extern "C" int vxm_conv3d_tcs_fwd_acc(const void* xa, const void* xb, const void* wpk, const float* bias, void* out, void* out_lo,
                                      const float* acc_in, int B, int D, int H, int W, int Ca, int Cb, int up, int Cout, int coutp,
                                      int kd, int out_mode, float slope, void* stream) {
  VXM_REQUIRE(out_mode >= 1 && out_mode <= 3, "conv3d_tcs_fwd_acc: out_mode must be 1 (fp32 planar), 2 (fp32 partial sums) or 3 (bf16 hi/lo pair)");
  VXM_REQUIRE(out_mode != 3 || out_lo, "conv3d_tcs_fwd_acc: out_mode 3 needs out_lo");
  return conv_tcs_launch(xa, xb, wpk, bias, out, nullptr, B, D, H, W, Ca, Cb, up, Cout, coutp, kd, out_mode, slope, nullptr, 0,
                         acc_in, out_lo, 0, 0, stream);
}

static int conv_tcs_launch(const void* xa, const void* xb, const void* wpk, const float* bias, void* out, const void* mask,
                           int B, int D, int H, int W, int Ca, int Cb, int up, int Cout, int coutp, int kd, int out_mode,
                           float slope, void* out2, int csplit, const float* acc_in, void* out_lo, int opitch, int poly,
                           void* stream) {
  VXM_REQUIRE(B > 0 && D > 0 && H > 0 && W > 0 && wpk && out, "conv3d_tcs_fwd: bad argument");
  VXM_REQUIRE(kd == 1 || kd == 3, "conv3d_tcs_fwd: kd must be 1 or 3");
  VXM_REQUIRE(coutp == 16 || coutp == 32 || coutp == 48 || coutp == 64, "conv3d_tcs_fwd: padded Cout must be 16, 32, 48 or 64");
  VXM_REQUIRE(!out2 || (out_mode == 0 && csplit > 0 && csplit < Cout && csplit % 8 == 0 && !mask), "conv3d_tcs_fwd: bad output split");
  VXM_REQUIRE(Cout > 0 && Cout <= coutp && (out_mode == 1 || out_mode == 2 || Cout % 8 == 0), "conv3d_tcs_fwd: unsupported Cout %d", Cout);
  VXM_REQUIRE(vxm_conv3d_tcs_supported(Ca, Cb, Cout), "conv3d_tcs_fwd: channel counts (%d,%d)->%d unsupported", Ca, Cb, Cout);
  VXM_REQUIRE((Ca == 0 || xa) && (Cb == 0 || xb), "conv3d_tcs_fwd: missing source tensor");
  VXM_REQUIRE(!up || (H % 2 == 0 && W % 2 == 0 && (kd == 1 || D % 2 == 0)), "conv3d_tcs_fwd: upsampled source needs even sizes");
  VXM_REQUIRE(poly == 0 || (kd == 3 && coutp == 32 && Cout == 32 && out_mode == 0 && !out2 && !acc_in && !opitch &&
                            (poly == 1 ? up && Ca == 32 && Cb == 16 && bias && !mask && slope >= 0.f && slope <= 1.f
                                       : !up && Ca == 32 && Cb == 0 && !bias && mask && D % 2 == 0 && H % 2 == 0 && W % 2 == 0)),
              "conv3d_tcs_poly: no polyphase mode %d kernel for (%d,%d)->%d", poly, Ca, Cb, Cout);
  ConvSArgs a{};
  const int cin = Ca + Cb;
  int g0, g1;
  groups_of(cin, &g0, &g1);
  a.xa = (const __nv_bfloat16*)xa; a.xb = (const __nv_bfloat16*)xb; a.wpk = (const __nv_bfloat16*)wpk; a.bias = bias;
  a.out = out; a.mask = (const __nv_bfloat16*)mask; a.out2 = out2; a.csplit = csplit;
  a.acc_in = acc_in; a.out_lo = out_lo;
  a.B = B; a.D = D; a.H = H; a.W = W; a.Ca = Ca; a.Cb = Cb; a.up = up; a.upd = (up && kd == 3) ? 1 : 0;
  a.Cout = Cout; a.out_mode = out_mode; a.slope = slope; a.opitch = opitch;
  VXM_REQUIRE(!opitch || (!out2 && out_mode != 1 && kd == 3 && coutp == 32 && ((g0 == 64 && g1 == 0) || (g0 == 32 && g1 == 16))),
              "conv3d_tcs_fwd: no blocked kernel for (%d,%d)->%d/%d, kd %d", Ca, Cb, Cout, coutp, kd);
  a.wbytes = (uint32_t)(poly ? poly_bytes(poly) : vxm_conv3d_tcs_packed_bytes(cin, coutp, kd));
  const size_t fixed = fixed_smem(a.wbytes);
  int HTv = 4;
  {
    const size_t slab8 = (size_t)10 * WT * (g0 + g1) * 2;
    const int ns8 = (int)((227 * 1024 - fixed) / slab8);
    if (g0 <= 32 && coutp <= 32 && ns8 >= (kd == 3 ? 5 : 3) && H > 4 && !opitch) HTv = 8;
    if (poly) HTv = poly == 2 ? 8 : 4;
  }
  a.tiles_h = (H + HTv - 1) / HTv; a.tiles_w = (W + WUSE - 1) / WUSE;
  int nsm = conv_ctas();
  const long long tiles = (long long)B * a.tiles_h * a.tiles_w;
  const int Do = poly == 2 ? D / 2 : D;
  a.dchunk = depth_chunk(Do, tiles, nsm, poly == 2 ? 1.25 : (kd == 3 ? 2.5 : 0.5), 40);
  a.nchunks = (Do + a.dchunk - 1) / a.dchunk;
  a.nitems = (int)(tiles * a.nchunks);
  const size_t slab = (size_t)(HTv + 2) * WT * (g0 + g1) * 2;
  int nslot = (int)((227 * 1024 - fixed) / slab);
  if (nslot > MAXSLOT) nslot = MAXSLOT;
  VXM_REQUIRE(nslot >= 4, "conv3d_tcs_fwd: not enough shared memory for the slab ring");
  a.nslot = nslot;
  size_t smem = fixed + (size_t)nslot * slab;
  int grid = a.nitems < nsm ? a.nitems : nsm;
  cudaStream_t st = as_stream(stream);
  if (poly != 2 && plan_tma(a, g0, g1, HTv) != 0) return VXM_ERR_CUDA;
  const bool acc_epi = acc_in != nullptr || out_mode >= 2;
  int epi = 0;
  {
    const char* e = getenv("VXM_B200_TCS_EPI");
    const bool spec = !acc_epi && !(e && e[0] == '0');
    const bool plain = spec && out_mode == 0 && Cout == coutp && (kd == 3 || coutp <= 32);
    if (plain && !out2 && !mask && slope >= 0.f && slope <= 1.f) epi = 1;
    else if (plain && !out2 && mask && !bias) epi = 2;
    else if (plain && kd == 3 && !mask && !bias && slope < 0.f && (!out2 || csplit % 16 == 0)) epi = 3;
    else if (spec && out_mode == 1 && !out2 && coutp <= 32 && g0 <= 32 && g1 == 0) epi = 4;
    if (poly) epi = poly;
  }
#define VXM_TCS_LAUNCH_E(KD_, G0_, G1_, CO_, HT_, ACC_, E_, ...)                                                                  \
  do {                                                                                                                            \
    VXM_CUDA(cudaFuncSetAttribute(conv_tcs_kernel<KD_, G0_, G1_, CO_, HT_, ACC_, E_, ##__VA_ARGS__>,                              \
                                  cudaFuncAttributeMaxDynamicSharedMemorySize, (int)smem));                                       \
    conv_tcs_kernel<KD_, G0_, G1_, CO_, HT_, ACC_, E_, ##__VA_ARGS__><<<grid, NTHREADS, smem, st>>>(a);                           \
  } while (0)
#define VXM_TCS_LAUNCH_OP(G0_, G1_)                                                                                               \
  do {                                                                                                                            \
    if (acc_epi) VXM_TCS_LAUNCH_E(3, G0_, G1_, 32, 4, true, 0, true);                                                             \
    else if (epi == 1) VXM_TCS_LAUNCH_E(3, G0_, G1_, 32, 4, false, 1, true);                                                      \
    else if (epi == 2) VXM_TCS_LAUNCH_E(3, G0_, G1_, 32, 4, false, 2, true);                                                      \
    else if (epi == 3) VXM_TCS_LAUNCH_E(3, G0_, G1_, 32, 4, false, 3, true);                                                      \
    else VXM_TCS_LAUNCH_E(3, G0_, G1_, 32, 4, false, 0, true);                                                                    \
  } while (0)
#define VXM_TCS_KD1(KD_, CO_) ((KD_) == 3 || (CO_) <= 32)
#define VXM_TCS_PL(G0_, G1_, CO_) ((CO_) <= 32 && (G0_) <= 32 && (G1_) == 0)
#define VXM_TCS_LAUNCH(KD_, G0_, G1_, CO_, HT_)                                                                                   \
  do {                                                                                                                            \
    if (acc_epi) VXM_TCS_LAUNCH_E(KD_, G0_, G1_, CO_, HT_, true, 0);                                                              \
    else if (VXM_TCS_KD1(KD_, CO_) && epi == 1) VXM_TCS_LAUNCH_E(KD_, G0_, G1_, CO_, HT_, false, VXM_TCS_KD1(KD_, CO_) ? 1 : 0);  \
    else if (VXM_TCS_KD1(KD_, CO_) && epi == 2) VXM_TCS_LAUNCH_E(KD_, G0_, G1_, CO_, HT_, false, VXM_TCS_KD1(KD_, CO_) ? 2 : 0);  \
    else if (KD_ == 3 && epi == 3) VXM_TCS_LAUNCH_E(3, G0_, G1_, CO_, HT_, false, 3);                                             \
    else if (VXM_TCS_PL(G0_, G1_, CO_) && epi == 4) VXM_TCS_LAUNCH_E(KD_, G0_, G1_, CO_, HT_, false, VXM_TCS_PL(G0_, G1_, CO_) ? 4 : 0); \
    else VXM_TCS_LAUNCH_E(KD_, G0_, G1_, CO_, HT_, false, 0);                                                                     \
  } while (0)
#define VXM_TCS_G8(KD_, CO_)                                                  \
  do {                                                                        \
    if (g0 == 16) VXM_TCS_LAUNCH(KD_, 16, 0, CO_, 8);                         \
    else if (g0 == 32 && g1 == 0) VXM_TCS_LAUNCH(KD_, 32, 0, CO_, 8);         \
    else VXM_TCS_LAUNCH(KD_, 32, 16, CO_, 8);                                 \
  } while (0)
#define VXM_TCS_G(KD_, CO_)                                                   \
  do {                                                                        \
    if (g0 == 16) VXM_TCS_LAUNCH(KD_, 16, 0, CO_, 4);                         \
    else if (g0 == 32 && g1 == 0) VXM_TCS_LAUNCH(KD_, 32, 0, CO_, 4);         \
    else if (g0 == 32) VXM_TCS_LAUNCH(KD_, 32, 16, CO_, 4);                   \
    else VXM_TCS_LAUNCH(KD_, 64, 0, CO_, 4);                                  \
  } while (0)
  if (poly) {
    if (poly == 1) VXM_TCS_LAUNCH_E(3, 32, 16, 32, 4, false, 1, false, 1);
    else VXM_TCS_LAUNCH_E(3, 32, 0, 32, 8, false, 2, false, 2);
  } else if (opitch) {
    if (g0 == 64) VXM_TCS_LAUNCH_OP(64, 0); else VXM_TCS_LAUNCH_OP(32, 16);
  } else if (HTv == 8) {
    if (kd == 3) { if (coutp == 16) VXM_TCS_G8(3, 16); else VXM_TCS_G8(3, 32); }
    else { if (coutp == 16) VXM_TCS_G8(1, 16); else VXM_TCS_G8(1, 32); }
  } else if (kd == 3) { if (coutp == 16) VXM_TCS_G(3, 16); else if (coutp == 32) VXM_TCS_G(3, 32); else if (coutp == 48) VXM_TCS_G(3, 48); else VXM_TCS_G(3, 64); }
  else { if (coutp == 16) VXM_TCS_G(1, 16); else if (coutp == 32) VXM_TCS_G(1, 32); else if (coutp == 48) VXM_TCS_G(1, 48); else VXM_TCS_G(1, 64); }
  return check_launch("conv3d_tcs_fwd");
}
```

voxelmorph_b200/engine_bf16.py:

```python
import torch

from . import _lib, tc

_weights_epoch = 0


def bump_weights_epoch():
    global _weights_epoch
    _weights_epoch += 1


class _Layer:
    __slots__ = ("w", "bias", "slope", "role", "a", "b", "out", "up", "ca", "cb", "cin", "cout", "fwd", "fwd_x3", "dgrad", "khm",
                 "dgrad_skip", "dgrad_img", "pk_fwd", "pk_dgrad", "pk_dgrad_skip", "pk_hi", "pk_lo", "w_hi", "w_lo", "srcs")


def _refuse(what):
    raise _lib.VxmError("bf16 tensor-core engine: %s (use VXM_B200_CONV_ENGINE=f32 for other U-Net shapes)" % what)


def _form(ca, cb, nout, kd, kw, split=None):
    blocks = tc.conv_blocks(ca, cb, nout, kd, split)
    launches = [(ca, cb, nout)] if blocks is None else \
        [((ca, cb) if src == 2 else (kb, 0)) + (nb,) for src, _, kb in blocks[0] for _, nb, _, _ in blocks[1]]
    for c0, c1, n in launches:
        if not _lib.load().vxm_conv3d_tcs_supported(c0, c1, n):
            _refuse("no tensor-core kernel takes a (%d + %d) -> %d convolution" % (c0, c1, n))
    return blocks if blocks is not None else tc.one_block(kw, nout)


def _walk(model):
    unet = model.unet_model
    w0 = unet.encoder[0][0].main.weight
    if w0.dim() not in (4, 5):
        _refuse("2-D or 3-D convolutions only")
    kd = 3 if w0.dim() == 5 else 1
    fold = kd == 3 and tc.kdfold_enabled()
    poly = kd == 3 and tc.polyphase_enabled()
    ops = []
    chans = [8]
    cur, pending_up, skips = 0, None, [None]

    def conv(m, slope, role="inner", extra=None):
        nonlocal cur, pending_up
        L = _Layer()
        L.w, L.bias, L.slope, L.role = m.weight, m.bias, slope, role
        if not isinstance(m.weight, torch.nn.Parameter):
            L.w, L.bias = m.weight.detach(), m.bias.detach()
        L.srcs = (L.w,) if extra is None else (m.weight, m.bias, extra.weight, extra.bias)
        L.a, L.b = pending_up if pending_up is not None else (cur, None)
        L.up, pending_up = pending_up is not None, None
        L.ca, L.cb = chans[L.a], (0 if L.b is None else chans[L.b])
        L.cout, L.cin = m.weight.shape[0] + (0 if extra is None else extra.weight.shape[0]), m.weight.shape[1]
        if m.weight.dim() != w0.dim():
            _refuse("convolutions of different dimensionality")
        if role == "first":
            if L.cin > 8:
                _refuse("the first convolution takes at most 8 input feature planes (src_feats + trg_feats)")
        elif L.ca + L.cb != L.cin or L.cin % 16 or L.cin > (64 if role == "flow" else 128):
            _refuse("unsupported convolution input channels %d (+%d); need a multiple of 16, at most 128 (64 into the flow "
                    "head)" % (L.ca, L.cb))
        if role == "flow" and L.cout > 8:
            _refuse("the flow head has %d components" % L.cout)
        if role != "flow" and L.cout not in (8, 16, 32, 64):
            _refuse("a U-Net convolution has %d output channels; supported feature counts are 8, 16, 32 and 64" % L.cout)
        L.fwd = L.fwd_x3 = _form(L.ca, L.cb, L.cout, kd, L.cin)
        if role == "first" and fold and 3 * L.cin <= 8 and L.cout in (8, 16, 32):
            L.fwd = "fold"
        L.dgrad_img = None
        if role == "first":
            L.dgrad = None
            L.dgrad_img = _form(L.cout, 0, L.cin, kd, L.cout)
        elif role == "flow" and fold and L.b is None and L.cin in (8, 16) and 3 * L.cout <= 16:
            L.dgrad = "fold"
        else:
            L.dgrad = _form(8 if role == "flow" else L.cout, 0, L.cin, kd, L.cout, L.ca if L.b is not None else None)
        L.dgrad_skip = None
        if poly and L.up and L.b is not None and L.ca == 32 and L.cout == 32:
            if L.cb == 16:
                L.fwd = ("poly", 1, L.ca)
            L.dgrad = ("poly", 2, L.ca)
            L.dgrad_skip = (((2, 0, L.cout),), ((L.ca, L.cb, 0, 0),))
            _form(L.cout, 0, L.cb, kd, L.cout)
        L.khm = L.cout <= 16
        L.out = cur = len(chans)
        chans.append(L.cout)
        ops.append(L)

    def pool():
        nonlocal cur
        ops.append(("pool", cur, len(chans)))
        cur = len(chans)
        chans.append(chans[ops[-1][1]])

    for convs in unet.encoder:
        for blk in convs:
            conv(blk.main, blk.activation.negative_slope, "first" if cur == 0 else "inner")
        skips.append(cur)
        pool()
    for level, convs in enumerate(unet.decoder):
        for blk in convs:
            conv(blk.main, blk.activation.negative_slope)
        if not unet.half_res or level < (unet.nb_levels - 2):
            pending_up = (cur, skips.pop())
    for blk in unet.remaining:
        conv(blk.main, blk.activation.negative_slope)
    conv(model.flow, None, "flow", getattr(model, "log_sigma", None))
    return ops


def supports(model):
    try:
        ops = _walk(model)
    except (AttributeError, _lib.VxmError):
        return False
    return all(L.role == "flow" or (L.cout in (8, 16, 32) and L.ca + L.cb <= 64) for L in ops if isinstance(L, _Layer))


class _Plan:

    def __init__(self, model):
        self.ops = _walk(model)
        self.layers = [L for L in self.ops if isinstance(L, _Layer)]
        self.nd = self.layers[0].w.dim() - 2
        for L in self.layers:
            if len(L.srcs) > 1:
                L.w = torch.empty((L.cout,) + tuple(L.w.shape[1:]), dtype=torch.float32, device=L.w.device)
                L.bias = torch.empty(L.cout, dtype=torch.float32, device=L.w.device)
        self.slope = {L.out: float(L.slope) for L in self.layers if L.slope is not None}
        bf16, x3 = [], []
        for L in self.layers:
            w = L.w.detach()
            L.w_hi, L.w_lo = torch.empty_like(w), torch.empty_like(w)
            bf16 += [(w, False, L.fwd)] + ([(w, True, L.dgrad)] if L.dgrad is not None else []) + \
                    ([(w, True, L.dgrad_skip)] if L.dgrad_skip is not None else [])
            x3 += [(L.w_hi, False, L.fwd_x3), (L.w_lo, False, L.fwd_x3)]
        self.bf16, self.x3 = tc.PackTable(bf16), tc.PackTable(x3)
        packs, packs3 = iter(self.bf16.packs), iter(self.x3.packs)
        for L in self.layers:
            L.pk_fwd, L.pk_dgrad = next(packs), (next(packs) if L.dgrad is not None else None)
            L.pk_dgrad_skip = next(packs) if L.dgrad_skip is not None else None
            L.pk_hi, L.pk_lo = next(packs3), next(packs3)
        self.ptrs = self.weight_ptrs()
        self.stamps = [None, None]
        self.img_table, self.img_stamp = None, None
        self.gen_ptr = None

    def weight_ptrs(self):
        return tuple(p.data_ptr() for L in self.layers for p in L.srcs)

    def refresh(self, split):
        stamp = (_weights_epoch, tuple(p._version for L in self.layers for p in L.srcs))
        if stamp != self.stamps[0]:
            for L in self.layers:
                if len(L.srcs) > 1:
                    fw, fb, lw, lb = L.srcs
                    torch.cat([fw.detach(), lw.detach()], out=L.w)
                    torch.cat([fb.detach(), lb.detach()], out=L.bias)
            self.bf16.refresh()
            self.stamps[0] = stamp
        if split and stamp != self.stamps[1]:
            for L in self.layers:
                w = L.w.detach()
                L.w_hi.copy_(w.to(torch.bfloat16))
                torch.sub(w, L.w_hi, out=L.w_lo)
            self.x3.refresh()
            self.stamps[1] = stamp

    def image_dgrad_packs(self):
        first = self.layers[0]
        if self.img_table is None:
            self.img_table = tc.PackTable([(first.w.detach(), True, first.dgrad_img)])
        stamp = (_weights_epoch, first.w._version)
        if stamp != self.img_stamp:
            self.img_table.refresh()
            self.img_stamp = stamp
        return self.img_table.packs[0]


def _plan_of(model, split, generated=None):
    plan = model.__dict__.get("_vxm_pack_plan")
    gen_ptr = None if generated is None else generated.data_ptr()
    if plan is None or plan.ptrs != plan.weight_ptrs() or plan.gen_ptr != gen_ptr:
        plan = _Plan(model)
        plan.gen_ptr = gen_ptr
        object.__setattr__(model, "_vxm_pack_plan", plan)
    plan.refresh(split)
    return plan


def _pool(x, nd):
    lib = _lib.load()
    B, D, H, W, C = x.shape
    Dc = D // 2 if nd == 3 else D
    y = torch.empty((B, Dc, H // 2, W // 2, C), dtype=torch.bfloat16, device=x.device)
    if (nd == 3 and D % 2) or H % 2 or W % 2:
        raise _lib.VxmError("bf16 engine: odd sizes cannot be pooled (U-Net shapes must be divisible by 2 per level)")
    _lib.check(lib.vxm_pool2_ndhwc_bf16(_lib.ptr(x), _lib.ptr(y), B, Dc, H // 2, W // 2, C, nd, _lib.stream_ptr()), "vxm_pool2_ndhwc_bf16")
    return y


def _sumpool_mask(g_fine, act_coarse, nd, slope):
    lib = _lib.load()
    B, Dc, Hc, Wc, C = act_coarse.shape
    out = torch.empty_like(act_coarse)
    _lib.check(lib.vxm_sumpool_mask_ndhwc_bf16(_lib.ptr(g_fine), _lib.ptr(act_coarse), _lib.ptr(out), B, Dc, Hc, Wc, C, nd, slope,
                                               _lib.stream_ptr()), "vxm_sumpool_mask_ndhwc_bf16")
    return out


def _unpool_combine(e_fine, g_skip, g_pool, nd, slope, e_lo=None):
    lib = _lib.load()
    B, D, H, W, C = e_fine.shape
    Dc = D // 2 if nd == 3 else D
    out = torch.empty_like(e_fine)
    if e_lo is None:
        _lib.check(lib.vxm_unpool_combine_ndhwc_bf16(_lib.ptr(e_fine), _lib.ptr(g_skip), _lib.ptr(g_pool), _lib.ptr(out), B, Dc, H // 2,
                                                     W // 2, C, nd, slope, _lib.stream_ptr()), "vxm_unpool_combine_ndhwc_bf16")
    else:
        _lib.check(lib.vxm_unpool_combine_split_ndhwc_bf16(_lib.ptr(e_fine), _lib.ptr(e_lo), _lib.ptr(g_skip), _lib.ptr(g_pool),
                                                           _lib.ptr(out), B, Dc, H // 2, W // 2, C, nd, slope, _lib.stream_ptr()),
                   "vxm_unpool_combine_split_ndhwc_bf16")
    return out


def _run(form, packs, xa, xb, nout, kd, bias=None, lo=None, **kw):
    if form[0] == "poly":
        wpk = packs[0, 0][0]
        return tc.conv_fwd_poly(xa, xb, wpk, bias, nout, kw["slope"]) if form[1] == 1 else tc.dgrad_poly(xa, wpk, kw["mask"], kw["slope"])
    if form == "fold" or (lo is None and len(form[0]) == len(form[1]) == 1):
        wpk, coutp = packs[0, 0]
        return tc.conv_fwd_t(xa, xb, wpk, (coutp, "s"), bias, nout, 1 if form == "fold" else kd, **kw)
    return tc.conv_fwd_blocked(xa, xb, form, packs, bias, nout, kd, lo=lo, **kw)


def _flat_grads(L):
    return all(getattr(p, "_vxm_flat_grad", False) and p.grad is not None and p.grad.is_contiguous()
               for p in (L.w, L.bias) if p is not None)


def forward_tape(model, source, target, split=False, generated=None):
    nd = source.dim() - 2
    kd = 3 if nd == 3 else 1
    _lib.require_cuda(source, target, what="VxmDense")
    source, target = _lib.contig(source), _lib.contig(target)
    plan = _plan_of(model, split, generated)
    planes = [source[:, i:i + 1] for i in range(source.shape[1])] + [target[:, i:i + 1] for i in range(target.shape[1])]
    first = plan.layers[0]
    if nd != plan.nd or len(planes) != first.cin:
        raise _lib.VxmError("bf16 engine: the model takes %d %d-D image planes (src_feats + trg_feats), got %d %d-D"
                            % (first.cin, plan.nd, len(planes), nd))
    tensors = {}
    lows = {}
    pool_lows = {}
    if split:
        tensors[0], lows[0] = tc.planar_to_ndhwc8_split(planes)
    elif first.fwd == "fold":
        tensors[0] = tc.planar_fold_kd(planes, 8)
    else:
        tensors[0] = tc.planar_to_ndhwc8(planes)
    for L in plan.ops:
        if not isinstance(L, _Layer):
            _, src, dst = L
            if split:
                tensors[dst], lows[dst] = tc.pool_split((tensors[src], lows[src]), nd)
                pool_lows[src] = lows[src]
            else:
                tensors[dst] = _pool(tensors[src], nd)
            continue
        bias = None if L.bias is None else L.bias.detach()
        kw = dict(up=L.up, slope=L.slope, out_fp32_planar=L.role == "flow")
        if split:
            out = _run(L.fwd_x3, L.pk_hi, tensors[L.a], tensors.get(L.b), L.cout, kd, bias, lo=(lows[L.a], lows.get(L.b), L.pk_lo), **kw)
        else:
            out = _run(L.fwd, L.pk_fwd, tensors[L.a], tensors.get(L.b), L.cout, kd, bias, **kw)
        if L.role == "flow":
            flow = out
        elif split:
            tensors[L.out], lows[L.out] = out
        else:
            tensors[L.out] = out
    if nd == 2:
        flow = flow.squeeze(2)
    return flow, dict(plan=plan, tensors=tensors, split=split, pool_lows=pool_lows,
                      generated=None if generated is None else generated.detach())


def backward_tape(ctx, g_flow, image_grad=False):
    plan, tensors = ctx["plan"], ctx["tensors"]
    nd = plan.nd
    kd = 3 if nd == 3 else 1
    g_flow = _lib.contig(g_flow.float())
    if nd == 2:
        g_flow = g_flow.unsqueeze(2)
    dev = g_flow.device
    batch = tc.WgradBatch.get(dev)
    batch.reset()
    gz = {}
    graw = {}
    gskip = {}
    grads = {}
    folded = []
    heads = []
    base = ctx.get("generated")
    dW = None if base is None else torch.zeros(base.numel(), dtype=torch.float32, device=dev)
    gen = {}
    if dW is not None:
        for L in plan.layers:
            if L.role != "flow":
                ow, ob = [(t.data_ptr() - base.data_ptr()) // base.element_size() for t in (L.w, L.bias)]
                gen[L] = (dW[ow:ow + L.w.numel()].view(L.w.shape), dW[ob:ob + L.cout])
        grads["generated"] = dW
    for L in reversed(plan.ops):
        if not isinstance(L, _Layer):
            _, src, dst = L
            gz[src] = _unpool_combine(tensors[src], gskip.pop(src, None), graw.pop(dst), nd, plan.slope[src], ctx["pool_lows"].pop(src, None))
            continue
        xa, xb = tensors[L.a], tensors.get(L.b)
        if L.role == "flow":
            planes = [g_flow[:, i:i + 1] for i in range(g_flow.shape[1])]
            g_in = tc.planar_fold_kd(planes, 16) if L.dgrad == "fold" else tc.planar_to_ndhwc8(planes)
        else:
            g_in = gz.pop(L.out)
        if L.dgrad == "fold":
            gwf = torch.empty((3 * nd, L.cin, 1, 3, 3), dtype=torch.float32, device=dev)
            gbf = torch.empty(3 * nd, dtype=torch.float32, device=dev) if L.bias is not None else None
            batch.add_khm(xa, g_in, gwf, gbf, L.cin, 3 * nd)
            folded.append((L, gwf, gbf))
        elif L.fwd == "fold" and not ctx["split"]:
            gwf = torch.empty((L.cout, 3 * L.cin, 1, 3, 3), dtype=torch.float32, device=dev)
            gbf = torch.empty(L.cout, dtype=torch.float32, device=dev) if L.bias is not None else None
            if L.khm:
                batch.add_khm(xa, g_in, gwf, gbf, 3 * L.cin, L.cout)
            else:
                batch.add(xa, None, g_in, gwf, gbf, 3 * L.cin, L.cout, 1, False, False)
            folded.append((L, gwf, gbf))
        elif L in gen:
            tc.conv_wgrad(xa, xb, g_in, L.cin, L.cout, kd, up=L.up, out_w=gen[L][0], out_b=gen[L][1], batch=batch)
        elif len(L.srcs) > 1:
            heads.append((L,) + tc.conv_wgrad(xa, xb, g_in, L.cin, L.cout, kd, up=L.up, batch=batch))
        elif _flat_grads(L):
            tc.conv_wgrad(xa, xb, g_in, L.cin, L.cout, kd, up=L.up, out_w=L.w.grad, out_b=None if L.bias is None else L.bias.grad,
                          batch=batch)
        else:
            gw, gb = tc.conv_wgrad(xa, xb, g_in, L.cin, L.cout, kd, up=L.up, batch=batch)
            grads[L.w] = gw.squeeze(2) if nd == 2 else gw
            if L.bias is not None:
                grads[L.bias] = gb
        if L.dgrad is None:
            if image_grad and L.role == "first":
                grads["images"] = _run(L.dgrad_img, plan.image_dgrad_packs(), g_in, None, L.cin, kd, out_fp32_planar=True)
            continue
        t = L.a
        if L.b is None:
            sl = plan.slope.get(t)
            res = _run(L.dgrad, L.pk_dgrad, g_in, None, L.cin, kd, slope=sl, mask=None if sl is None else tensors[t])
            (graw if sl is None else gz)[t] = res
        elif L.dgrad_skip is not None:
            gz[t] = _run(L.dgrad, L.pk_dgrad, g_in, None, L.ca, kd, mask=tensors[t], slope=plan.slope[t])
            gskip[L.b] = _run(L.dgrad_skip, L.pk_dgrad_skip, g_in, None, L.cb, kd)
        else:
            g_up, g_sk = _run(L.dgrad, L.pk_dgrad, g_in, None, L.cin, kd, split=L.ca)
            gz[t] = _sumpool_mask(g_up, tensors[t], nd, plan.slope[t])
            del g_up
            gskip[L.b] = g_sk
    batch.flush()
    for L, gwf, gbf in folded:
        gw, gb = (unfold_grad_first(gwf, L.cout, L.cin), gbf) if L.role == "first" else unfold_grad_flow(gwf, gbf, nd, L.cin)
        if L in gen:
            gen[L][0].add_(gw)
            gen[L][1].add_(gb)
        elif _flat_grads(L):
            L.w.grad.add_(gw)
            if L.bias is not None:
                L.bias.grad.add_(gb)
        else:
            grads[L.w] = gw.contiguous()
            if L.bias is not None:
                grads[L.bias] = gb.contiguous()
    for L, gw, gb in heads:
        fw, fb, lw, lb = L.srcs
        k = fw.shape[0]
        gw = gw.squeeze(2) if nd == 2 else gw
        for p, g in ((fw, gw[:k]), (fb, gb[:k]), (lw, gw[k:]), (lb, gb[k:])):
            if getattr(p, "_vxm_flat_grad", False) and p.grad is not None and p.grad.is_contiguous():
                p.grad.add_(g)
            else:
                grads[p] = g.contiguous()
    return grads



def fold_planes(planes):
    x = torch.cat(planes, dim=1)
    xp = torch.nn.functional.pad(x, (0, 0, 0, 0, 1, 1))
    D = x.shape[2]
    return torch.cat([xp[:, :, kd:kd + D] for kd in range(3)], dim=1).permute(0, 2, 3, 4, 1).contiguous()


def fold_weight_first(w):
    co, p = w.shape[0], w.shape[1]
    return w.permute(0, 2, 1, 3, 4).reshape(co, 3 * p, 3, 3)


def fold_weight_flow_dgrad(w):
    c, ci = w.shape[0], w.shape[1]
    return w.flip(2, 3, 4).permute(1, 2, 0, 3, 4).reshape(ci, 3 * c, 3, 3)


def unfold_grad_first(gwf, cout, cin):
    return gwf.view(cout, 3, cin, 3, 3).permute(0, 2, 1, 3, 4)


def unfold_grad_flow(gwf, gbf, nd, cin):
    gw = gwf.view(3, nd, cin, 3, 3).flip(0).permute(1, 2, 0, 3, 4)
    return gw, (None if gbf is None else gbf[nd:2 * nd])


class _UnetFlowFn(torch.autograd.Function):
    @staticmethod
    def forward(ctx, model, source, target, split, generated, *params):
        flow, tape = forward_tape(model, source, target, split=split, generated=generated)
        ctx.tape = tape
        ctx.params = params
        ctx.model_ref = model
        ctx.image_grads = tuple(ctx.needs_input_grad[1:3])
        ctx.src_feats = source.shape[1]
        return flow

    @staticmethod
    def backward(ctx, g_flow):
        dp = getattr(ctx.model_ref, "_dp", None)
        if dp is not None:
            dp.schedule()
        grads = backward_tape(ctx.tape, g_flow, image_grad=any(ctx.image_grads))
        ctx.tape = None
        g_source = g_target = None
        if any(ctx.image_grads):
            g_img = grads.pop("images")
            if g_flow.dim() == 4:
                g_img = g_img.squeeze(2)
            if ctx.image_grads[0]:
                g_source = g_img[:, :ctx.src_feats]
            if ctx.image_grads[1]:
                g_target = g_img[:, ctx.src_feats:]
        return (None, g_source, g_target, None, grads.get("generated")) + tuple(grads.get(p) for p in ctx.params)


def unet_flow(model, source, target, split=False, generated=None):
    head = [model.flow] + ([model.log_sigma] if hasattr(model, "log_sigma") else [])
    params = list(model.unet_model.parameters()) + [p for m in head for p in m.parameters()]
    return _UnetFlowFn.apply(model, source, target, bool(split), generated, *params)
```

voxelmorph_b200/tc.py:

```python
import ctypes
import functools
import threading

import torch

from . import _lib


def np_for(cout):
    if cout <= 16:
        return 16
    if cout <= 32:
        return 32
    if cout <= 48:
        return 48
    if cout <= 64:
        return 64
    raise _lib.VxmError("tensor-core conv engine: at most 64 output channels per launch (got %d)" % cout)


def to_ndhwc_bf16(x):
    return x.permute(0, 2, 3, 4, 1).contiguous().to(torch.bfloat16)


def from_ndhwc(x):
    return x.permute(0, 4, 1, 2, 3).float().contiguous()


def pack_weights(w, transposed=False):
    lib = _lib.load()
    if w.dim() == 4:
        w = w.unsqueeze(2)
    w = w.contiguous()
    Cout, Cin, kd = w.shape[0], w.shape[1], w.shape[2]
    cin_eff, nout = (Cout, Cin) if transposed else (Cin, Cout)
    NP = np_for(nout)
    nbytes = int(lib.vxm_conv3d_tc_packed_bytes(cin_eff, NP, kd))
    out = torch.empty(nbytes // 2, dtype=torch.bfloat16, device=w.device)
    _lib.check(lib.vxm_conv3d_tc_pack(_lib.ptr(w), _lib.ptr(out), Cout, Cin, kd, NP, 1 if transposed else 0,
                                      _lib.stream_ptr()), "vxm_conv3d_tc_pack")
    return out, NP


def conv_fwd(xa, xb, wpk, NP, bias, cout, kd, up=False, planar=None, out_fp32_planar=False, slope=None, mask=None, split=None):
    lib = _lib.load()
    if planar is not None:
        ref = planar[0]
        B, D, H, W = ref.shape[0], ref.shape[-3] if ref.dim() == 5 else 1, ref.shape[-2], ref.shape[-1]
        arr_p = (ctypes.c_void_p * 4)(*([p.data_ptr() for p in planar] + [0] * (4 - len(planar))))
        arr_s = (ctypes.c_longlong * 4)(*([p.stride(0) for p in planar] + [0] * (4 - len(planar))))
        xf, xs, npl, Ca, Cb = arr_p, arr_s, len(planar), 0, 0
        dev = ref.device
    else:
        full = xb if xb is not None else xa
        B, D, H, W = full.shape[0], full.shape[1], full.shape[2], full.shape[3]
        if xb is None and up:
            D, H, W = (D * 2 if kd == 3 else D), H * 2, W * 2
        Ca = 0 if xa is None else xa.shape[-1]
        Cb = 0 if xb is None else xb.shape[-1]
        xf, xs, npl = None, None, 0
        dev = full.device
    out2 = None
    if out_fp32_planar:
        out = torch.empty((B, cout, D, H, W), dtype=torch.float32, device=dev)
    elif split:
        out = torch.empty((B, D, H, W, split), dtype=torch.bfloat16, device=dev)
        out2 = torch.empty((B, D, H, W, cout - split), dtype=torch.bfloat16, device=dev)
    else:
        out = torch.empty((B, D, H, W, cout), dtype=torch.bfloat16, device=dev)
    s = -1.0 if slope is None else float(slope)
    _lib.check(lib.vxm_conv3d_tc_fwd(_lib.ptr(xa), _lib.ptr(xb), xf, xs, npl, _lib.ptr(wpk), _lib.ptr(bias), _lib.ptr(out),
                                     _lib.ptr(mask), B, D, H, W, Ca, Cb, 1 if up else 0, cout, NP, kd,
                                     1 if out_fp32_planar else 0, s, _lib.ptr(out2), int(split or 0), _lib.stream_ptr()),
               "vxm_conv3d_tc_fwd")
    return (out, out2) if split else out


def _planar_args(planar):
    if planar is None:
        return None, None, 0
    arr_p = (ctypes.c_void_p * 4)(*([p.data_ptr() for p in planar] + [0] * (4 - len(planar))))
    arr_s = (ctypes.c_longlong * 4)(*([p.stride(0) for p in planar] + [0] * (4 - len(planar))))
    return arr_p, arr_s, len(planar)


_wgrad_ws = {}
_ws_lock = threading.Lock()


def conv_wgrad(xa, xb, gz, cin, cout, kd, up=False, planar_x=None, planar_g=None, need_bias=True, out_w=None, out_b=None, batch=None):
    lib = _lib.load()
    ref = gz if gz is not None else planar_g[0]
    dev = ref.device
    accumulate = out_w is not None
    gw = out_w if accumulate else torch.empty((cout, cin, kd, 3, 3), dtype=torch.float32, device=dev)
    gb = out_b if accumulate else (torch.empty(cout, dtype=torch.float32, device=dev) if need_bias else None)
    if batch is not None:
        batch.add(xa, xb, gz, gw, gb, cin, cout, kd, up, accumulate)
        return gw, gb
    if gz is not None:
        B, D, H, W, Cg = gz.shape
    else:
        B, D, H, W, Cg = ref.shape[0], (ref.shape[-3] if ref.dim() == 5 else 1), ref.shape[-2], ref.shape[-1], 8
    key = (dev.index, torch.cuda.current_stream(dev).cuda_stream, kd)
    work = _wgrad_ws.get(key)
    if work is None:
        with _ws_lock:
            work = _wgrad_ws.get(key)
            if work is None:
                work = torch.empty(int(lib.vxm_conv3d_tc_wgrad_workspace_bytes(kd)), dtype=torch.uint8, device=dev)
                _wgrad_ws[key] = work
    xf, xs, npx = _planar_args(planar_x)
    gf, gs, npg = _planar_args(planar_g)
    Ca = 0 if xa is None else xa.shape[-1]
    Cb = 0 if xb is None else xb.shape[-1]
    _lib.check(lib.vxm_conv3d_tc_wgrad(_lib.ptr(xa), _lib.ptr(xb), xf, xs, npx, _lib.ptr(gz), gf, gs, npg, _lib.ptr(gw),
                                       _lib.ptr(gb), _lib.ptr(work), B, D, H, W, Ca, Cb, 1 if up else 0, cin, Cg, cout, kd,
                                       1 if accumulate else 0, _lib.stream_ptr()), "vxm_conv3d_tc_wgrad")
    return gw, gb


def planar_to_ndhwc8(planes):
    lib = _lib.load()
    ref = planes[0]
    B = ref.shape[0]
    D, H, W = (ref.shape[-3] if ref.dim() == 5 else 1), ref.shape[-2], ref.shape[-1]
    n = len(planes)
    arr_p = (ctypes.c_void_p * 8)(*([p.data_ptr() for p in planes] + [0] * (8 - n)))
    arr_s = (ctypes.c_longlong * 8)(*([p.stride(0) for p in planes] + [0] * (8 - n)))
    out = torch.empty((B, D, H, W, 8), dtype=torch.bfloat16, device=ref.device)
    _lib.check(lib.vxm_planar_to_ndhwc8_bf16(arr_p, arr_s, n, _lib.ptr(out), B, D * H * W, _lib.stream_ptr()),
               "vxm_planar_to_ndhwc8_bf16")
    return out


def kdfold_enabled():
    import os
    return os.environ.get("VXM_B200_KDFOLD", "1") != "0"


def polyphase_enabled():
    import os
    return os.environ.get("VXM_B200_POLYPHASE", "1") != "0"


def pack_weights_poly(w, mode, ca):
    table = PackTable([(w.contiguous(), mode == 2, ("poly", mode, ca))])
    table.refresh()
    torch.cuda.current_stream(w.device).synchronize()
    return table.packs[0][0, 0][0]


def conv_fwd_poly(xa, xb, wpk, bias, cout, slope):
    lib = _lib.load()
    B, D, H, W = xb.shape[:4]
    out = torch.empty((B, D, H, W, cout), dtype=torch.bfloat16, device=xb.device)
    _lib.check(lib.vxm_conv3d_tcs_poly(_lib.ptr(xa), _lib.ptr(xb), _lib.ptr(wpk), _lib.ptr(bias), _lib.ptr(out), None, B, D, H, W,
                                       xa.shape[-1], xb.shape[-1], cout, 1, float(slope), _lib.stream_ptr()), "vxm_conv3d_tcs_poly")
    return out


def dgrad_poly(g, wpk, act, slope):
    lib = _lib.load()
    B, D, H, W, C = g.shape
    out = torch.empty_like(act)
    _lib.check(lib.vxm_conv3d_tcs_poly(_lib.ptr(g), None, _lib.ptr(wpk), None, _lib.ptr(out), _lib.ptr(act), B, D, H, W, C, 0,
                                       act.shape[-1], 2, float(slope), _lib.stream_ptr()), "vxm_conv3d_tcs_poly")
    return out


def planar_fold_kd(planes, cout):
    lib = _lib.load()
    ref = planes[0]
    B, D, H, W = ref.shape[0], ref.shape[-3], ref.shape[-2], ref.shape[-1]
    n = len(planes)
    arr_p = (ctypes.c_void_p * 8)(*([p.data_ptr() for p in planes] + [0] * (8 - n)))
    arr_s = (ctypes.c_longlong * 8)(*([p.stride(0) for p in planes] + [0] * (8 - n)))
    out = torch.empty((B, D, H, W, cout), dtype=torch.bfloat16, device=ref.device)
    _lib.check(lib.vxm_planar_fold_kd_bf16(arr_p, arr_s, n, _lib.ptr(out), B, D, H * W, cout, _lib.stream_ptr()), "vxm_planar_fold_kd_bf16")
    return out


def pack_weights_fold(w, transposed=False):
    table = PackTable([(w.contiguous(), transposed, "fold")])
    table.refresh()
    torch.cuda.current_stream(w.device).synchronize()
    out, coutp = table.packs[0][0, 0]
    return out, (coutp, "s")



def pack_weights_t(w, transposed=False, variant="s"):
    lib = _lib.load()
    if w.dim() == 4:
        w = w.unsqueeze(2)
    w = w.contiguous()
    Cout, Cin, kd = w.shape[0], w.shape[1], w.shape[2]
    cin_eff, nout = (Cout, Cin) if transposed else (Cin, Cout)
    coutp = 16 if nout <= 16 else (32 if nout <= 32 else (48 if nout <= 48 else 64))
    fb, fp = (lib.vxm_conv3d_tcs_packed_bytes, lib.vxm_conv3d_tcs_pack) if variant == "s" else \
             (lib.vxm_conv3d_tct_packed_bytes, lib.vxm_conv3d_tct_pack)
    nbytes = int(fb(cin_eff, coutp, kd))
    out = torch.empty(nbytes // 2, dtype=torch.bfloat16, device=w.device)
    _lib.check(fp(_lib.ptr(w), _lib.ptr(out), Cout, Cin, kd, coutp, 1 if transposed else 0, _lib.stream_ptr()),
               "vxm_conv3d_tc%s_pack" % variant)
    return out, (coutp, variant)


def conv_fwd_t(xa, xb, wpk, coutp, bias, cout, kd, up=False, out_fp32_planar=False, slope=None, mask=None, split=None):
    lib = _lib.load()
    coutp, variant = coutp if isinstance(coutp, tuple) else (coutp, "t")
    fwd = lib.vxm_conv3d_tcs_fwd if variant == "s" else lib.vxm_conv3d_tct_fwd
    full = xb if xb is not None else xa
    B, D, H, W = full.shape[0], full.shape[1], full.shape[2], full.shape[3]
    if xb is None and up:
        D, H, W = (D * 2 if kd == 3 else D), H * 2, W * 2
    Ca = 0 if xa is None else xa.shape[-1]
    Cb = 0 if xb is None else xb.shape[-1]
    dev = full.device
    out2 = None
    if out_fp32_planar:
        out = torch.empty((B, cout, D, H, W), dtype=torch.float32, device=dev)
    elif split:
        out = torch.empty((B, D, H, W, split), dtype=torch.bfloat16, device=dev)
        out2 = torch.empty((B, D, H, W, cout - split), dtype=torch.bfloat16, device=dev)
    else:
        out = torch.empty((B, D, H, W, cout), dtype=torch.bfloat16, device=dev)
    s = -1.0 if slope is None else float(slope)
    _lib.check(fwd(_lib.ptr(xa), _lib.ptr(xb), _lib.ptr(wpk), _lib.ptr(bias), _lib.ptr(out), _lib.ptr(mask),
                   B, D, H, W, Ca, Cb, 1 if up else 0, cout, coutp, kd, 1 if out_fp32_planar else 0, s,
                   _lib.ptr(out2), int(split or 0), _lib.stream_ptr()), "vxm_conv3d_tc%s_fwd" % variant)
    return (out, out2) if split else out



@functools.lru_cache(maxsize=None)
def conv_blocks(ca, cb, nout, kd, split=None):
    lib = _lib.load()
    cin = ca + cb
    if cin <= 64 and nout <= 64 and lib.vxm_conv3d_tcs_fits(cin, np_for(nout), kd):
        return None
    if cin <= 64:
        ks = ((2, 0, cin),)
    else:
        ks = ((0, 0, ca), (1, ca, cb))
        if ca == 64 and cb != 64:
            ks = ks[::-1]
    nbmax = 64 if lib.vxm_conv3d_tcs_fits(max(k[2] for k in ks), 64, kd) else 32
    pieces = [(0, split, 0), (split, nout - split, 1)] if split else [(0, nout, 0)]
    return ks, tuple((p0 + j, min(nbmax, pn - j), dst, j) for p0, pn, dst in pieces for j in range(0, pn, nbmax))


def one_block(cin, nout):
    return ((2, 0, cin),), ((0, nout, 0, 0),)


class PackTable:

    def __init__(self, operands):
        lib = _lib.load()
        dsz = int(lib.vxm_conv3d_tcs_pack_desc_bytes())
        host = ctypes.create_string_buffer(dsz * sum(1 if f == "fold" or f[0] == "poly" else len(f[0]) * len(f[1]) for _, _, f in operands))
        self.packs, self.n, self.total = [], 0, 0
        for w, transposed, form in operands:
            w5 = w if w.dim() == 5 else w.unsqueeze(2)
            Cout, Cin, kd = w5.shape[0], w5.shape[1], w5.shape[2]
            t = 1 if transposed else 0
            packs = {}
            if form != "fold" and form[0] == "poly":
                _, mode, ca = form
                out = torch.empty(int(lib.vxm_conv3d_tcs_poly_packed_bytes(mode, Cout, Cin, ca)) // 2, dtype=torch.bfloat16, device=w.device)
                cnt = lib.vxm_conv3d_tcs_pack_desc_poly(self._slot(host, dsz), _lib.ptr(w5), _lib.ptr(out), Cout, Cin, ca, mode, self.total)
                self._add(packs, (0, 0), out, 32, cnt)
            elif form == "fold":
                real_in, nout = (Cout, Cin) if transposed else (Cin, Cout)
                coutp = 16 if nout <= 16 else 32
                out = torch.empty(int(lib.vxm_conv3d_tcs_packed_bytes(3 * real_in, coutp, 1)) // 2, dtype=torch.bfloat16, device=w.device)
                cnt = lib.vxm_conv3d_tcs_pack_desc_fold(self._slot(host, dsz), _lib.ptr(w5), _lib.ptr(out), Cout, Cin, coutp, t, self.total)
                self._add(packs, (0, 0), out, coutp, cnt)
            else:
                for ki, (_, k0, kb) in enumerate(form[0]):
                    for ni, (n0, nb, _, _) in enumerate(form[1]):
                        coutp = np_for(nb)
                        out = torch.empty(int(lib.vxm_conv3d_tcs_packed_bytes(kb, coutp, kd)) // 2, dtype=torch.bfloat16, device=w.device)
                        cnt = lib.vxm_conv3d_tcs_pack_desc_blk(self._slot(host, dsz), _lib.ptr(w5), _lib.ptr(out), Cout, Cin, kd, coutp, t,
                                                               n0, nb, k0, kb, self.total)
                        self._add(packs, (ki, ni), out, coutp, cnt)
            self.packs.append(packs)
        self.descs = torch.frombuffer(bytearray(host.raw), dtype=torch.uint8).to(operands[0][0].device)

    def _slot(self, host, dsz):
        return ctypes.cast(ctypes.addressof(host) + self.n * dsz, ctypes.c_void_p)

    def _add(self, packs, key, out, coutp, cnt):
        if cnt <= 0:
            raise _lib.VxmError("vxm_conv3d_tcs_pack_desc: %s" % _lib.last_error())
        packs[key] = (out, coutp)
        self.n, self.total = self.n + 1, self.total + cnt

    def refresh(self):
        _lib.check(_lib.load().vxm_conv3d_tcs_pack_multi(_lib.ptr(self.descs), self.n, self.total, _lib.stream_ptr()),
                   "vxm_conv3d_tcs_pack_multi")


def pack_weights_blocks(w, transposed, blocks):
    table = PackTable([(w.contiguous(), transposed, blocks)])
    table.refresh()
    packs = table.packs[0]
    packs[None] = table
    return packs


def _ptr_at(t, off):
    return None if t is None else ctypes.c_void_p(t.data_ptr() + off * t.element_size())


def conv_fwd_blocked(xa, xb, blocks, packs, bias, nout, kd, up=False, slope=None, mask=None, split=None, lo=None, out_fp32_planar=False):
    lib = _lib.load()
    ks, ns = blocks
    full = xb if xb is not None else xa
    B, D, H, W = full.shape[0], full.shape[1], full.shape[2], full.shape[3]
    if xb is None and up:
        D, H, W = (D * 2 if kd == 3 else D), H * 2, W * 2
    if mask is not None and split:
        raise _lib.VxmError("conv_fwd_blocked: a mask with a split output is not implemented")
    if out_fp32_planar and (split or len(ns) != 1):
        raise _lib.VxmError("conv_fwd_blocked: the fp32 planar output takes one N block")
    if out_fp32_planar:
        outs = [torch.empty((B, nout, D, H, W), dtype=torch.float32, device=full.device)]
    else:
        outs = [torch.empty((B, D, H, W, c), dtype=torch.bfloat16, device=full.device) for c in ([split, nout - split] if split else [nout])]
    outs_lo = [torch.empty_like(o) for o in outs] if lo is not None and not out_fp32_planar else [None] * len(outs)
    s = -1.0 if slope is None else float(slope)
    ca = 0 if xa is None else xa.shape[-1]
    cb = 0 if xb is None else xb.shape[-1]
    for ni, (n0, nb, dst, doff) in enumerate(ns):
        out, pitch = outs[dst], outs[dst].shape[-1]
        passes = [(ki, 0, False) for ki in range(len(ks))] if lo is None else \
                 [p for ki in range(len(ks)) for p in ((ki, 1, False), (ki, 0, True), (ki, 0, False))]
        acc = None
        for pi, (ki, xlo, wlo) in enumerate(passes):
            src, _, kb = ks[ki]
            pa = xa if not xlo else lo[0]
            pb = xb if not xlo else lo[1]
            if src == 0:
                x0, x1, c0, c1, u = pa, None, kb, 0, up
            elif src == 1:
                x0, x1, c0, c1, u = pb, None, kb, 0, False
            else:
                x0, x1, c0, c1, u = pa, pb, ca, cb, up
            wpk, coutp = (lo[2] if wlo else packs)[(ki, ni)]
            if pi + 1 < len(passes):
                ain = acc
                if acc is None:
                    acc = torch.empty((B, D, H, W, coutp), dtype=torch.float32, device=full.device)
                o, olo, m, mode, op, bptr = _lib.ptr(acc), None, None, 2, 0, None
            elif out_fp32_planar:
                _lib.check(lib.vxm_conv3d_tcs_fwd_acc(_lib.ptr(x0), _lib.ptr(x1), _lib.ptr(wpk), _lib.ptr(bias), _lib.ptr(out), None,
                                                      _lib.ptr(acc), B, D, H, W, c0, c1, 1 if u else 0, nb, coutp, kd, 1, s,
                                                      _lib.stream_ptr()), "vxm_conv3d_tcs_fwd_acc")
                continue
            else:
                ain = acc
                o, olo, m = _ptr_at(out, doff), _ptr_at(outs_lo[dst], doff), _ptr_at(mask, n0)
                mode, op, bptr = (3 if lo is not None else 0), pitch, _ptr_at(bias, n0)
            _lib.check(lib.vxm_conv3d_tcs_fwd_blk(_lib.ptr(x0), _lib.ptr(x1), _lib.ptr(wpk), bptr, o, olo, m, _lib.ptr(ain),
                                                  B, D, H, W, c0, c1, 1 if u else 0, nb, coutp, kd, mode, s, op, _lib.stream_ptr()),
                       "vxm_conv3d_tcs_fwd_blk")
    if out_fp32_planar:
        return outs[0]
    if lo is not None:
        return outs[0], outs_lo[0]
    return tuple(outs) if split else outs[0]



def planar_to_ndhwc8_split(planes):
    lib = _lib.load()
    ref = planes[0]
    B = ref.shape[0]
    D, H, W = (ref.shape[-3] if ref.dim() == 5 else 1), ref.shape[-2], ref.shape[-1]
    n = len(planes)
    arr_p = (ctypes.c_void_p * 8)(*([p.data_ptr() for p in planes] + [0] * (8 - n)))
    arr_s = (ctypes.c_longlong * 8)(*([p.stride(0) for p in planes] + [0] * (8 - n)))
    hi = torch.empty((B, D, H, W, 8), dtype=torch.bfloat16, device=ref.device)
    lo = torch.empty_like(hi)
    _lib.check(lib.vxm_planar_to_ndhwc8_split_bf16(arr_p, arr_s, n, _lib.ptr(hi), _lib.ptr(lo), B, D * H * W, _lib.stream_ptr()),
               "vxm_planar_to_ndhwc8_split_bf16")
    return hi, lo


def pool_split(x, nd):
    lib = _lib.load()
    xh, xl = x
    B, D, H, W, C = xh.shape
    Dc = D // 2 if nd == 3 else D
    yh = torch.empty((B, Dc, H // 2, W // 2, C), dtype=torch.bfloat16, device=xh.device)
    yl = torch.empty_like(yh)
    _lib.check(lib.vxm_pool2_split_ndhwc_bf16(_lib.ptr(xh), _lib.ptr(xl), _lib.ptr(yh), _lib.ptr(yl), B, Dc, H // 2, W // 2, C, nd,
                                              _lib.stream_ptr()), "vxm_pool2_split_ndhwc_bf16")
    return yh, yl



class WgradBatch:

    _cache = {}
    WORK_BYTES = 512 << 20

    @classmethod
    def get(cls, device):
        key = (device.index, torch.cuda.current_stream(device).cuda_stream)
        b = cls._cache.get(key)
        if b is None:
            with _ws_lock:
                b = cls._cache.get(key)
                if b is None:
                    b = cls._cache[key] = cls(device)
        return b

    def __init__(self, device):
        lib = _lib.load()
        self.dev = device
        self.dsz = int(lib.vxm_conv3d_tc_wgrad2_desc_bytes())
        self.maxn = int(lib.vxm_conv3d_tc_wgrad2_max_pending())
        self.host = ctypes.create_string_buffer(self.dsz * self.maxn)
        self.n = ctypes.c_int(0)
        self.used = ctypes.c_size_t(0)
        self.off = 0
        self.work = torch.empty(self.WORK_BYTES, dtype=torch.uint8, device=device)

    def add(self, xa, xb, gz, gw, gb, cin, cout, kd, up, accumulate):
        lib = _lib.load()
        B, D, H, W, Cg = gz.shape
        Ca = 0 if xa is None else xa.shape[-1]
        Cb = 0 if xb is None else xb.shape[-1]
        nsub = ((Ca + 31) // 32 + (Cb + 31) // 32) * ((Cg + 31) // 32)
        need = int(lib.vxm_conv3d_tc_wgrad2_partial_bytes(kd)) * ((nsub + 1) // 2)
        if self.off + need > self.WORK_BYTES or self.n.value + max(2, nsub) > self.maxn:
            self.flush()
        _lib.check(lib.vxm_conv3d_tc_wgrad2_partial(_lib.ptr(xa), _lib.ptr(xb), _lib.ptr(gz), _lib.ptr(gw), _lib.ptr(gb),
                                                    ctypes.c_void_p(self.work.data_ptr() + self.off), self.WORK_BYTES - self.off,
                                                    ctypes.byref(self.used), ctypes.cast(self.host, ctypes.c_void_p), ctypes.byref(self.n),
                                                    B, D, H, W, Ca, Cb, 1 if up else 0, cin, Cg, cout, kd, 1 if accumulate else 0,
                                                    _lib.stream_ptr()), "vxm_conv3d_tc_wgrad2_partial")
        self.off += int(self.used.value)

    def add_khm(self, x, gz, gw2d, gb, cin_real, cout_real):
        lib = _lib.load()
        need = int(lib.vxm_conv3d_tc_wgrad2_partial_bytes(1))
        if self.off + need > self.WORK_BYTES or self.n.value + 1 > self.maxn:
            self.flush()
        B, D, H, W, Cg = gz.shape
        _lib.check(lib.vxm_conv3d_tc_wgrad2_partial_khm(_lib.ptr(x), _lib.ptr(gz), _lib.ptr(gw2d), _lib.ptr(gb),
                                                        ctypes.c_void_p(self.work.data_ptr() + self.off), self.WORK_BYTES - self.off,
                                                        ctypes.byref(self.used), ctypes.cast(self.host, ctypes.c_void_p), ctypes.byref(self.n),
                                                        B, D, H, W, x.shape[-1], cin_real, Cg, cout_real, 0, _lib.stream_ptr()),
                   "vxm_conv3d_tc_wgrad2_partial_khm")
        self.off += int(self.used.value)

    def reset(self):
        self.n.value = 0
        self.off = 0

    def flush(self):
        if self.n.value:
            _lib.check(_lib.load().vxm_conv3d_tc_wgrad2_flush(ctypes.cast(self.host, ctypes.c_void_p), self.n.value, _lib.stream_ptr()),
                       "vxm_conv3d_tc_wgrad2_flush")
        self.n.value = 0
        self.off = 0
```

Measured before the change: 85.99.

## Fold flow-head depth taps into padded outputs for 16-channel kd=1 conv

Adds an output-folded forward path for the 16->3 flow head conv. The three depth taps become extra output columns of a kd=1 tensor-core GEMM, and the results are accumulated across consecutive depth slices in registers, with W-seam exchange through shared memory and shuffles. This replaces a full kd=3 conv on a tiny 3-channel output with one kd=1 MMA over 16 padded outputs per group, cutting wasted MMA work and weight loads. It adds a new epilogue, a special weight pack, and two extra pipeline iterations per depth chunk, with some risk of correctness errors at the seams.

Measured after the change: 87.59 (median of 6 runs). 1.9% higher.

```diff
diff --git a/include/vxm_b200.h b/include/vxm_b200.h
--- a/include/vxm_b200.h
+++ b/include/vxm_b200.h
@@ -117,6 +117,8 @@
 int vxm_conv3d_tcs_fwd(const void* xa, const void* xb, const void* wpk, const float* bias, void* out, const void* mask,
                        int B, int D, int H, int W, int Ca, int Cb, int up, int Cout, int coutp, int kd, int out_mode,
                        float slope, void* out2, int csplit, void* stream);
+int vxm_conv3d_tcs_fwd_fold_out(const void* x, const void* wpk, const float* bias, void* out, int B, int D, int H, int W, int Cin,
+                                int Cout, int Ctot, void* stream);
 int vxm_conv3d_tcs_fwd_acc(const void* xa, const void* xb, const void* wpk, const float* bias, void* out, void* out_lo,
                            const float* acc_in, int B, int D, int H, int W, int Ca, int Cb, int up, int Cout, int coutp,
                            int kd, int out_mode, float slope, void* stream);
diff --git a/voxelmorph_b200/_lib.py b/voxelmorph_b200/_lib.py
--- a/voxelmorph_b200/_lib.py
+++ b/voxelmorph_b200/_lib.py
@@ -63,6 +63,7 @@
     "vxm_conv3d_tcs_pack_desc_fold": (c_i, [c_f, c_f, c_f] + [c_i] * 5),
     "vxm_conv3d_tcs_pack_multi": (c_i, [c_f, c_i, c_i, c_f]),
     "vxm_conv3d_tcs_fwd": (c_i, [c_f, c_f, c_f, c_f, c_f, c_f] + [c_i] * 11 + [c_fl, c_f, c_i, c_f]),
+    "vxm_conv3d_tcs_fwd_fold_out": (c_i, [c_f] * 4 + [c_i] * 7 + [c_f]),
     "vxm_conv3d_tcs_fwd_acc": (c_i, [c_f, c_f, c_f, c_f, c_f, c_f, c_f] + [c_i] * 11 + [c_fl, c_f]),
     "vxm_conv3d_tcs_fits": (c_i, [c_i] * 3),
     "vxm_conv3d_tcs_fwd_blk": (c_i, [c_f] * 8 + [c_i] * 11 + [c_fl, c_i, c_f]),
diff --git a/voxelmorph_b200/csrc/conv3d_tc_s.cu b/voxelmorph_b200/csrc/conv3d_tc_s.cu
--- a/voxelmorph_b200/csrc/conv3d_tc_s.cu
+++ b/voxelmorph_b200/csrc/conv3d_tc_s.cu
@@ -48,7 +48,10 @@
   static_assert(PD != 1 || G1 > 0, "the polyphase forward merges channel group 0 and keeps group 1");
   static_assert(PD != 2 || (G1 == 0 && COUT == 32 && HT == 8 && EPI == 2), "the coarse dgrad: 32 -> 32 channels, 8-row tiles");
   static_assert(EPI != 4 || (PD == 0 && !ACC && !OP && COUT <= 32), "the fp32 planar epilogue drains in the fragment layout");
-  static_assert(KD == 3 || EPI == 0 || (EPI != 3 && COUT <= 32), "KD = 1: fragment-layout epilogues 1, 2, 4 only");
+  static_assert(KD == 3 || EPI == 0 || (EPI != 3 && COUT <= 32), "KD = 1: fragment-layout epilogues 1, 2, 4, 5 only");
+  constexpr bool FO = EPI == 5;
+  static_assert(!FO || (KD == 1 && G0 == 16 && G1 == 0 && COUT == 16 && HT == 8 && !ACC && !OP && PD == 0),
+                "kd folded into the outputs: 16 input channels, 16 padded outputs, 8-row tiles");
   constexpr int SROWS = (HT + 2) * WT;
   constexpr int NH = PD == 2 ? 1 : HT / 4;
   constexpr int NEVEN = (HT + 3) / 2;
@@ -105,7 +108,7 @@
       const int wt = item % a.tiles_w, ht = (item / a.tiles_w) % a.tiles_h;
       const int ch = (item / HW_tiles) % a.nchunks, b = item / (HW_tiles * a.nchunks);
       const int h0 = ht * HT, w0 = wt * WUSE, d0 = ch * a.dchunk, d1 = min(d0 + a.dchunk, Dout);
-      const int s_begin = PD == 2 ? 2 * d0 - 1 : (KD == 3 ? d0 - 1 : d0), s_end = PD == 2 ? 2 * d1 + 1 : (KD == 3 ? d1 + 1 : d1);
+      const int s_begin = PD == 2 ? 2 * d0 - 1 : (KD == 3 || FO ? d0 - 1 : d0), s_end = PD == 2 ? 2 * d1 + 1 : (KD == 3 || FO ? d1 + 1 : d1);
       int soff[KMAX];
       uint32_t doff[KMAX];
 #pragma unroll
@@ -239,7 +242,7 @@
         }
         cnt_base += last + 2;
       } else {
-        cnt_base += nd;
+        cnt_base += nd + (FO ? 2 : 0);
       }
     };
     if constexpr (EPI != 0) {
@@ -249,6 +252,7 @@
       const size_t HWp = (size_t)Ho * Wo;
       const int q = lane >> 2, p = lane & 3, half = wq & 1, pair = wq >> 1;
       const int xbar = 3 + 2 * grp + pair;
+      [[maybe_unused]] const float fo_bias = FO && a.bias && p < a.Cout ? __ldg(a.bias + p) : 0.f;
       constexpr bool ROWS = NSUB > 1 || PD == 2;
       constexpr int XPAIR = NF * 2 * COUT;
       static_assert(2 * 2 * XPAIR <= ACC_STAGE_FLOATS, "seam exchange fits the stage buffer");
@@ -258,7 +262,7 @@
       if constexpr (ORD) {
         for (int item = blockIdx.x; item < a.nitems; item += gridDim.x) {
           const int d0 = ((item / HW_tiles) % a.nchunks) * a.dchunk;
-          nev += (uint32_t)(min(d0 + a.dchunk, Dout) - d0) * NH;
+          nev += (uint32_t)(min(d0 + a.dchunk, Dout) - d0 + (FO ? 2 : 0)) * NH;
         }
         if (grp == 1) named_bar_arrive(7, 256);
       }
@@ -279,8 +283,10 @@
               if (wp + 8 * i >= 1 && wp + 8 * i <= WUSE && w + 8 * i < a.W && hbase + 4 * hb + 2 * blk < Ho)
                 okm |= 1u << (4 * hb + 2 * blk + i);
         size_t vbase = (((size_t)b * Dout + d0) * Ho + hbase) * Wo + (size_t)(long long)w;
-        [[maybe_unused]] const size_t DHWp = (size_t)Dout * HWp, pbase = (size_t)b * (a.Cout - 1) * DHWp;
-        for (int j = 0; j < nd; ++j) {
+        [[maybe_unused]] const size_t DHWp = (size_t)Dout * HWp, pbase = (size_t)b * ((FO && a.opitch ? a.opitch : a.Cout) - 1) * DHWp;
+        [[maybe_unused]] float pend0[FO ? 3 : 1][NF][2] = {}, pend1[FO ? 3 : 1][NF][2] = {};
+        [[maybe_unused]] float* const fo_out = FO ? reinterpret_cast<float*>(a.out) + pbase + (size_t)p * DHWp : nullptr;
+        for (int j = 0; j < nd + (FO ? 2 : 0); ++j) {
           const uint32_t js = PD == 2 ? 2u * j : (uint32_t)j;
           observe(cnt_base + js + (PD == 2 ? 3u : (KD == 3 ? 2u : 0u)));
           const uint32_t hslot = (cnt_base + js) % NSLOT;
@@ -321,6 +327,49 @@
               mma(hslot, hb, sub, acc, (d0 + j) & 1);
               if (ORD && e + 1 < nev) named_bar_arrive(8 - grp, 256);
               wg_wait<0>();
+              if constexpr (FO) {
+                float r[3][NF][2];
+#pragma unroll
+                for (int kw = 0; kw < 3; ++kw)
+#pragma unroll
+                  for (int f = 0; f < NF; ++f)
+#pragma unroll
+                    for (int i = 0; i < 2; ++i) {
+                      const int k = 4 * kw * (COUT / 8) + 2 * i;
+                      r[kw][f][i] = pend0[kw][f][i] + acc[f][k + 4];
+                      pend0[kw][f][i] = pend1[kw][f][i] + acc[f][k + 1];
+                      pend1[kw][f][i] = acc[f][k];
+                    }
+                if (j < 2) continue;
+                float* xb = stage + xpar * (2 * XPAIR) + pair * XPAIR;
+                xpar ^= 1u;
+#pragma unroll
+                for (int f = 0; f < NF; ++f) {
+                  if (half == 0 && q == 7) xb[f * 2 * COUT + 2 * p] = r[0][f][1];
+                  if (half == 1 && q == 0) xb[f * 2 * COUT + COUT + 2 * p] = r[2][f][0];
+                }
+                named_bar(xbar, 64);
+#pragma unroll
+                for (int f = 0; f < NF; ++f) {
+                  const float* xs = xb + f * 2 * COUT + 2 * p;
+                  const float a1 = __shfl_sync(0xffffffffu, q == 7 ? r[0][f][0] : r[0][f][1], (lane + 28) & 31);
+                  const float a0 = __shfl_sync(0xffffffffu, r[0][f][0], (lane + 28) & 31);
+                  const float b0 = __shfl_sync(0xffffffffu, q == 0 ? r[2][f][1] : r[2][f][0], (lane + 4) & 31);
+                  const float b1 = __shfl_sync(0xffffffffu, r[2][f][1], (lane + 4) & 31);
+                  float v[2];
+                  v[0] = q == 0 ? xs[0] : a0;
+                  v[0] += r[1][f][0];
+                  v[0] += b0;
+                  v[1] = a1;
+                  v[1] += r[1][f][1];
+                  v[1] += q == 7 ? xs[COUT] : b1;
+#pragma unroll
+                  for (int i = 0; i < 2; ++i)
+                    if (p < a.Cout && (okm >> (4 * hb + 2 * f + i) & 1u))
+                      fo_out[vox_of(f, i)] = v[i] + fo_bias;
+                }
+                continue;
+              }
               if constexpr (ROWS) {
                 const bool valid = rvalid;
                 const size_t vox = rvox;
@@ -446,7 +495,7 @@
               }
             }
           }
-          vbase += HWp;
+          if (!FO || j >= 2) vbase += HWp;
           if (lane == 0) {
             mbar_arrive(&empty[hslot]);
             if (PD == 2) mbar_arrive(&empty[(hslot + 1) % NSLOT]);
@@ -657,6 +706,9 @@
                                : d.w[((size_t)(d.k0 + ci) * d.Cin + d.n0 + co) * 27 + (26 - tp)];
           }
       }
+    } else if (d.fold < 0) {
+      const int fk = co < 8 ? co & 1 : 2, c = co < 8 ? co >> 1 : (co - 8) >> 1;
+      if (c < d.Cout && (co < 8 || !(co & 1)) && ci < d.Cin) v = d.w[((size_t)c * d.Cin + ci) * 27 + (fk * 3 + kh) * 3 + g];
     } else if (d.fold) {
       const int fk = ci / d.fold, c = ci % d.fold;
       const int tap3 = (fk * 3 + kh) * 3 + g;
@@ -757,6 +809,15 @@
 
 extern "C" int vxm_conv3d_tcs_pack_desc_fold(void* desc_host, const float* w, void* wpk, int Cout, int Cin, int coutp, int transposed, int begin) {
   VXM_REQUIRE(desc_host && w && wpk && Cout > 0 && Cin > 0 && (coutp == 16 || coutp == 32), "conv3d_tcs_pack_desc_fold: bad argument");
+  if (transposed == 2) {
+    VXM_REQUIRE(Cin == 16 && Cout <= 4 && coutp == 16, "conv3d_tcs_pack_desc_fold: no output-folded operand of a %d -> %d head", Cin, Cout);
+    PackDesc d;
+    d.w = w; d.out = (__nv_bfloat16*)wpk; d.Cout = Cout; d.Cin = Cin; d.KD = 1; d.COUT = 16; d.NN = 48; d.G0 = 16; d.G1 = 0;
+    d.transposed = 0; d.begin = begin; d.count = 3 * d.NN * 16; d.fold = -1;
+    d.n0 = d.nb = d.k0 = d.kb = 0; d.poly = 0;
+    memcpy(desc_host, &d, sizeof(d));
+    return d.count;
+  }
   const int real_in = transposed ? Cout : Cin, nout = transposed ? Cin : Cout;
   VXM_REQUIRE(3 * real_in <= 16 && nout <= coutp, "conv3d_tcs_pack_desc_fold: %d x 3 input channels / %d outputs do not fit", real_in, nout);
   int g0, g1;
@@ -814,13 +875,13 @@
 static int conv_tcs_launch(const void* xa, const void* xb, const void* wpk, const float* bias, void* out, const void* mask,
                            int B, int D, int H, int W, int Ca, int Cb, int up, int Cout, int coutp, int kd, int out_mode,
                            float slope, void* out2, int csplit, const float* acc_in, void* out_lo, int opitch, int poly,
-                           void* stream);
+                           int fold_out, void* stream);
 
 extern "C" int vxm_conv3d_tcs_poly(const void* xa, const void* xb, const void* wpk, const float* bias, void* out, const void* mask, int B,
                                    int D, int H, int W, int Ca, int Cb, int Cout, int mode, float slope, void* stream) {
   VXM_REQUIRE(mode == 1 || mode == 2, "conv3d_tcs_poly: mode must be 1 (forward) or 2 (coarse dgrad)");
   return conv_tcs_launch(xa, xb, wpk, bias, out, mask, B, D, H, W, Ca, Cb, mode == 1 ? 1 : 0, Cout, 32, 3, 0, slope, nullptr, 0,
-                         nullptr, nullptr, 0, mode, stream);
+                         nullptr, nullptr, 0, mode, 0, stream);
 }
 
 static size_t fixed_smem(uint32_t wbytes) { return ((wbytes + 1023u) & ~1023u) + NGRP * ACC_STAGE_FLOATS * sizeof(float) + 1024 + 512; }
@@ -837,7 +898,7 @@
                                   float slope, void* out2, int csplit, void* stream) {
   VXM_REQUIRE(out_mode == 0 || out_mode == 1, "conv3d_tcs_fwd: out_mode must be 0 (bf16 channels-last) or 1 (fp32 planar)");
   return conv_tcs_launch(xa, xb, wpk, bias, out, mask, B, D, H, W, Ca, Cb, up, Cout, coutp, kd, out_mode, slope, out2, csplit,
-                         nullptr, nullptr, 0, 0, stream);
+                         nullptr, nullptr, 0, 0, 0, stream);
 }
 
 extern "C" int vxm_conv3d_tcs_fwd_blk(const void* xa, const void* xb, const void* wpk, const float* bias, void* out, void* out_lo,
@@ -847,7 +908,7 @@
   VXM_REQUIRE(out_mode != 3 || out_lo, "conv3d_tcs_fwd_blk: out_mode 3 needs out_lo");
   VXM_REQUIRE(opitch == 0 || (opitch >= Cout && opitch % 8 == 0 && out_mode != 2), "conv3d_tcs_fwd_blk: bad output pitch %d", opitch);
   return conv_tcs_launch(xa, xb, wpk, bias, out, mask, B, D, H, W, Ca, Cb, up, Cout, coutp, kd, out_mode, slope, nullptr, 0,
-                         acc_in, out_lo, opitch == Cout ? 0 : opitch, 0, stream);
+                         acc_in, out_lo, opitch == Cout ? 0 : opitch, 0, 0, stream);
 }
 
 extern "C" int vxm_conv3d_tcs_fwd_acc(const void* xa, const void* xb, const void* wpk, const float* bias, void* out, void* out_lo,
@@ -856,13 +917,21 @@
   VXM_REQUIRE(out_mode >= 1 && out_mode <= 3, "conv3d_tcs_fwd_acc: out_mode must be 1 (fp32 planar), 2 (fp32 partial sums) or 3 (bf16 hi/lo pair)");
   VXM_REQUIRE(out_mode != 3 || out_lo, "conv3d_tcs_fwd_acc: out_mode 3 needs out_lo");
   return conv_tcs_launch(xa, xb, wpk, bias, out, nullptr, B, D, H, W, Ca, Cb, up, Cout, coutp, kd, out_mode, slope, nullptr, 0,
-                         acc_in, out_lo, 0, 0, stream);
+                         acc_in, out_lo, 0, 0, 0, stream);
+}
+
+extern "C" int vxm_conv3d_tcs_fwd_fold_out(const void* x, const void* wpk, const float* bias, void* out, int B, int D, int H, int W,
+                                           int Cin, int Cout, int Ctot, void* stream) {
+  VXM_REQUIRE(x && Cin == 16 && Cout >= 1 && Cout <= 4 && Ctot >= Cout, "conv3d_tcs_fwd_fold_out: a 16 -> (1 .. 4) head only, got %d -> %d of %d",
+              Cin, Cout, Ctot);
+  return conv_tcs_launch(x, nullptr, wpk, bias, out, nullptr, B, D, H, W, Cin, 0, 0, Cout, 16, 1, 1, -1.f, nullptr, 0, nullptr,
+                         nullptr, Ctot, 0, 1, stream);
 }
 
 static int conv_tcs_launch(const void* xa, const void* xb, const void* wpk, const float* bias, void* out, const void* mask,
                            int B, int D, int H, int W, int Ca, int Cb, int up, int Cout, int coutp, int kd, int out_mode,
                            float slope, void* out2, int csplit, const float* acc_in, void* out_lo, int opitch, int poly,
-                           void* stream) {
+                           int fold_out, void* stream) {
   VXM_REQUIRE(B > 0 && D > 0 && H > 0 && W > 0 && wpk && out, "conv3d_tcs_fwd: bad argument");
   VXM_REQUIRE(kd == 1 || kd == 3, "conv3d_tcs_fwd: kd must be 1 or 3");
   VXM_REQUIRE(coutp == 16 || coutp == 32 || coutp == 48 || coutp == 64, "conv3d_tcs_fwd: padded Cout must be 16, 32, 48 or 64");
@@ -875,6 +944,8 @@
                             (poly == 1 ? up && Ca == 32 && Cb == 16 && bias && !mask && slope >= 0.f && slope <= 1.f
                                        : !up && Ca == 32 && Cb == 0 && !bias && mask && D % 2 == 0 && H % 2 == 0 && W % 2 == 0)),
               "conv3d_tcs_poly: no polyphase mode %d kernel for (%d,%d)->%d", poly, Ca, Cb, Cout);
+  VXM_REQUIRE(!fold_out || (kd == 1 && coutp == 16 && Cout <= 4 && out_mode == 1 && Ca == 16 && Cb == 0 && !up && !mask && !out2 &&
+                            !acc_in && opitch >= Cout && !poly), "conv3d_tcs_fwd_fold_out: bad argument");
   ConvSArgs a{};
   const int cin = Ca + Cb;
   int g0, g1;
@@ -884,7 +955,7 @@
   a.acc_in = acc_in; a.out_lo = out_lo;
   a.B = B; a.D = D; a.H = H; a.W = W; a.Ca = Ca; a.Cb = Cb; a.up = up; a.upd = (up && kd == 3) ? 1 : 0;
   a.Cout = Cout; a.out_mode = out_mode; a.slope = slope; a.opitch = opitch;
-  VXM_REQUIRE(!opitch || (!out2 && out_mode != 1 && kd == 3 && coutp == 32 && ((g0 == 64 && g1 == 0) || (g0 == 32 && g1 == 16))),
+  VXM_REQUIRE(!opitch || fold_out || (!out2 && out_mode != 1 && kd == 3 && coutp == 32 && ((g0 == 64 && g1 == 0) || (g0 == 32 && g1 == 16))),
               "conv3d_tcs_fwd: no blocked kernel for (%d,%d)->%d/%d, kd %d", Ca, Cb, Cout, coutp, kd);
   a.wbytes = (uint32_t)(poly ? poly_bytes(poly) : vxm_conv3d_tcs_packed_bytes(cin, coutp, kd));
   const size_t fixed = fixed_smem(a.wbytes);
@@ -894,12 +965,13 @@
     const int ns8 = (int)((227 * 1024 - fixed) / slab8);
     if (g0 <= 32 && coutp <= 32 && ns8 >= (kd == 3 ? 5 : 3) && H > 4 && !opitch) HTv = 8;
     if (poly) HTv = poly == 2 ? 8 : 4;
+    if (fold_out) HTv = 8;
   }
   a.tiles_h = (H + HTv - 1) / HTv; a.tiles_w = (W + WUSE - 1) / WUSE;
   int nsm = conv_ctas();
   const long long tiles = (long long)B * a.tiles_h * a.tiles_w;
   const int Do = poly == 2 ? D / 2 : D;
-  a.dchunk = depth_chunk(Do, tiles, nsm, poly == 2 ? 1.25 : (kd == 3 ? 2.5 : 0.5), 40);
+  a.dchunk = depth_chunk(Do, tiles, nsm, poly == 2 ? 1.25 : (kd == 3 || fold_out ? 2.5 : 0.5), 40);
   a.nchunks = (Do + a.dchunk - 1) / a.dchunk;
   a.nitems = (int)(tiles * a.nchunks);
   const size_t slab = (size_t)(HTv + 2) * WT * (g0 + g1) * 2;
@@ -922,6 +994,7 @@
     else if (plain && kd == 3 && !mask && !bias && slope < 0.f && (!out2 || csplit % 16 == 0)) epi = 3;
     else if (spec && out_mode == 1 && !out2 && coutp <= 32 && g0 <= 32 && g1 == 0) epi = 4;
     if (poly) epi = poly;
+    if (fold_out) epi = 5;
   }
 #define VXM_TCS_LAUNCH_E(KD_, G0_, G1_, CO_, HT_, ACC_, E_, ...)                                                                  \
   do {                                                                                                                            \
@@ -964,6 +1037,8 @@
   if (poly) {
     if (poly == 1) VXM_TCS_LAUNCH_E(3, 32, 16, 32, 4, false, 1, false, 1);
     else VXM_TCS_LAUNCH_E(3, 32, 0, 32, 8, false, 2, false, 2);
+  } else if (epi == 5) {
+    VXM_TCS_LAUNCH_E(1, 16, 0, 16, 8, false, 5);
   } else if (opitch) {
     if (g0 == 64) VXM_TCS_LAUNCH_OP(64, 0); else VXM_TCS_LAUNCH_OP(32, 16);
   } else if (HTv == 8) {
diff --git a/voxelmorph_b200/engine_bf16.py b/voxelmorph_b200/engine_bf16.py
--- a/voxelmorph_b200/engine_bf16.py
+++ b/voxelmorph_b200/engine_bf16.py
@@ -75,6 +75,8 @@
             L.dgrad = "fold"
         else:
             L.dgrad = _form(8 if role == "flow" else L.cout, 0, L.cin, kd, L.cout, L.ca if L.b is not None else None)
+        if role == "flow" and fold and L.b is None and L.cin == 16:
+            L.fwd = "fold"
         L.dgrad_skip = None
         if poly and L.up and L.b is not None and L.ca == 32 and L.cout == 32:
             if L.cb == 16:
@@ -228,6 +230,8 @@
     if form[0] == "poly":
         wpk = packs[0, 0][0]
         return tc.conv_fwd_poly(xa, xb, wpk, bias, nout, kw["slope"]) if form[1] == 1 else tc.dgrad_poly(xa, wpk, kw["mask"], kw["slope"])
+    if form == "fold" and kw.get("out_fp32_planar"):
+        return tc.conv_fwd_fold_out(xa, [packs[k][0] for k in sorted(packs)], bias, nout)
     if form == "fold" or (lo is None and len(form[0]) == len(form[1]) == 1):
         wpk, coutp = packs[0, 0]
         return tc.conv_fwd_t(xa, xb, wpk, (coutp, "s"), bias, nout, 1 if form == "fold" else kd, **kw)
@@ -327,7 +331,7 @@
             gbf = torch.empty(3 * nd, dtype=torch.float32, device=dev) if L.bias is not None else None
             batch.add_khm(xa, g_in, gwf, gbf, L.cin, 3 * nd)
             folded.append((L, gwf, gbf))
-        elif L.fwd == "fold" and not ctx["split"]:
+        elif L.fwd == "fold" and L.role == "first" and not ctx["split"]:
             gwf = torch.empty((L.cout, 3 * L.cin, 1, 3, 3), dtype=torch.float32, device=dev)
             gbf = torch.empty(L.cout, dtype=torch.float32, device=dev) if L.bias is not None else None
             if L.khm:
@@ -406,6 +410,11 @@
 def fold_weight_flow_dgrad(w):
     c, ci = w.shape[0], w.shape[1]
     return w.flip(2, 3, 4).permute(1, 2, 0, 3, 4).reshape(ci, 3 * c, 3, 3)
+
+
+def fold_weight_flow_fwd(w):
+    c, ci = w.shape[0], w.shape[1]
+    return w.permute(2, 0, 1, 3, 4).reshape(3 * c, ci, 3, 3)
 
 
 def unfold_grad_first(gwf, cout, cin):
diff --git a/voxelmorph_b200/tc.py b/voxelmorph_b200/tc.py
--- a/voxelmorph_b200/tc.py
+++ b/voxelmorph_b200/tc.py
@@ -185,8 +185,28 @@
     table = PackTable([(w.contiguous(), transposed, "fold")])
     table.refresh()
     torch.cuda.current_stream(w.device).synchronize()
-    out, coutp = table.packs[0][0, 0]
+    packs = table.packs[0]
+    if len(packs) > 1:
+        return [packs[k][0] for k in sorted(packs)], (16, "s")
+    out, coutp = packs[0, 0]
     return out, (coutp, "s")
+
+
+def fold_out_groups(cout):
+    k = (cout + 3) // 4
+    n = (cout + k - 1) // k
+    return [(c0, min(n, cout - c0)) for c0 in range(0, cout, n)]
+
+
+def conv_fwd_fold_out(x, wpks, bias, cout):
+    lib = _lib.load()
+    B, D, H, W, C = x.shape
+    wpks = [wpks] if torch.is_tensor(wpks) else wpks
+    out = torch.empty((B, cout, D, H, W), dtype=torch.float32, device=x.device)
+    for wpk, (c0, n) in zip(wpks, fold_out_groups(cout)):
+        _lib.check(lib.vxm_conv3d_tcs_fwd_fold_out(_lib.ptr(x), _lib.ptr(wpk), _lib.ptr(bias[c0:]), _lib.ptr(out[:, c0]), B, D, H, W,
+                                                   C, n, cout, _lib.stream_ptr()), "vxm_conv3d_tcs_fwd_fold_out")
+    return out
 
 
 
@@ -255,12 +275,17 @@
     return ((2, 0, cin),), ((0, nout, 0, 0),)
 
 
+def _fold_out(w, transposed, form):
+    return form == "fold" and not transposed and 3 * w.shape[1] > 16
+
+
 class PackTable:
 
     def __init__(self, operands):
         lib = _lib.load()
         dsz = int(lib.vxm_conv3d_tcs_pack_desc_bytes())
-        host = ctypes.create_string_buffer(dsz * sum(1 if f == "fold" or f[0] == "poly" else len(f[0]) * len(f[1]) for _, _, f in operands))
+        host = ctypes.create_string_buffer(dsz * sum(len(fold_out_groups(w.shape[0])) if _fold_out(w, t, f) else
+                                                     1 if f == "fold" or f[0] == "poly" else len(f[0]) * len(f[1]) for w, t, f in operands))
         self.packs, self.n, self.total = [], 0, 0
         for w, transposed, form in operands:
             w5 = w if w.dim() == 5 else w.unsqueeze(2)
@@ -272,6 +297,11 @@
                 out = torch.empty(int(lib.vxm_conv3d_tcs_poly_packed_bytes(mode, Cout, Cin, ca)) // 2, dtype=torch.bfloat16, device=w.device)
                 cnt = lib.vxm_conv3d_tcs_pack_desc_poly(self._slot(host, dsz), _lib.ptr(w5), _lib.ptr(out), Cout, Cin, ca, mode, self.total)
                 self._add(packs, (0, 0), out, 32, cnt)
+            elif _fold_out(w, transposed, form):
+                for gi, (c0, nc) in enumerate(fold_out_groups(Cout)):
+                    out = torch.empty(int(lib.vxm_conv3d_tcs_packed_bytes(Cin, 16, 1)) // 2, dtype=torch.bfloat16, device=w.device)
+                    cnt = lib.vxm_conv3d_tcs_pack_desc_fold(self._slot(host, dsz), _lib.ptr(w5[c0:]), _lib.ptr(out), nc, Cin, 16, 2, self.total)
+                    self._add(packs, (0, gi), out, 16, cnt)
             elif form == "fold":
                 real_in, nout = (Cout, Cin) if transposed else (Cin, Cout)
                 coutp = 16 if nout <= 16 else 32
```
